# pranoyr/attention-models

Hardware: AMD Instinct MI355X
Metric: ViTVQGAN 256px train-step images/sec (higher is better)
Workload: dtype f32; 1 GPU; BASELINE.json configs[2]: ViTVQGAN dim=256 patch=8 img=256 depth=6+6 h=8 d=64 mlp=2048 (SwiGLU), codebook 8192x32; GAN train step (D phase + G phase, gradient penalty, per_loss_weight=0), Adam, clip 1.0; global_batch=32, batch_per_gpu=32, parallelism=dp1

## Files before the change

### attention-models_amd/amk/dense.py

```python
import ctypes

import torch

from . import lib as _lib
from .lib import EPI_BIAS, EPI_RESID, EPI_SWIGLU, EPI_SWIGLU_BWD, GEMM_NN, GEMM_NT, GEMM_TN, GemmDesc


def _p(t):
    return ctypes.c_void_p(t.data_ptr()) if t is not None else ctypes.c_void_p(0)


def _stream():
    return ctypes.c_void_p(torch.cuda.current_stream().cuda_stream)


def _mat(t, what):
    if t is None:
        return None
    if not t.is_cuda:
        raise RuntimeError("amk ops run only on MI355X (HIP) tensors; got a CPU tensor. There is no CPU fallback.")
    if t.dtype != torch.float32:
        raise RuntimeError(f"amk kernels compute in fp32; got {t.dtype} for {what}")
    if t.dim() != 2:
        raise RuntimeError(f"{what} must be a matrix, got shape {tuple(t.shape)}")
    if t.stride(1) != 1 or t.stride(0) % 4 or t.data_ptr() % 16:
        t = t.contiguous()
    return t


def _vec(t, n, what):
    if t is None:
        return None
    if not t.is_cuda or t.dtype != torch.float32:
        raise RuntimeError(f"{what}: an fp32 HIP tensor is required")
    t = t.contiguous()
    if t.numel() != n:
        raise RuntimeError(f"{what}: {t.numel()} elements, expected {n}")
    return t


def supported(*dims):
    return all(d > 0 and d % 4 == 0 for d in dims)


def _run(d, ws=None):
    L = _lib.load()
    rc = L.amk_gemm_f32(ctypes.byref(d), _p(ws), ws.numel() * 4 if ws is not None else 0, _stream())
    _lib.check(rc, "amk_gemm_f32")


def _set_ln(d, ln, M, K):
    if ln is None:
        return ()
    mean, rstd, gamma, beta = ln
    keep = (_vec(mean, M, "ln mean"), _vec(rstd, M, "ln rstd"), _vec(gamma, K, "ln gamma"), _vec(beta, K, "ln beta"))
    d.ln_mean, d.ln_rstd, d.ln_gamma, d.ln_beta = (_p(t) for t in keep)
    return keep


def row_stats(x2, eps=1e-5):
    x2 = _mat(x2, "x")
    M, D = x2.shape
    if x2.stride(0) != D:
        x2 = x2.contiguous()
    mean = torch.empty((M,), device=x2.device, dtype=torch.float32)
    rstd = torch.empty_like(mean)
    _lib.check(_lib.load().amk_row_stats(_p(x2), M, D, float(eps), _p(mean), _p(rstd), _stream()), "amk_row_stats")
    return mean, rstd


def gemm_nt(a, w, bias=None, *, w2=None, bias2=None, resid=None, ln=None, out=None):
    a, w, w2, resid = _mat(a, "a"), _mat(w, "w"), _mat(w2, "w2"), _mat(resid, "resid")
    M, K = a.shape
    N1 = w.shape[0]
    N2 = w2.shape[0] if w2 is not None else 0
    if w.shape[1] != K or (w2 is not None and w2.shape[1] != K):
        raise RuntimeError(f"gemm_nt: a {tuple(a.shape)} against w {tuple(w.shape)}")
    c = out if out is not None else torch.empty((M, N1), device=a.device, dtype=torch.float32)
    c2 = torch.empty((M, N2), device=a.device, dtype=torch.float32) if w2 is not None else None
    d = GemmDesc(op=GEMM_NT, epilogue=EPI_RESID if resid is not None else EPI_BIAS, m=M, n=N1 + N2, k=K,
                 split=N1 if w2 is not None else 0)
    bias, bias2 = _vec(bias, N1, "bias"), _vec(bias2, N2, "bias2")
    d.a, d.lda, d.w, d.ldw, d.c, d.ldc, d.bias = _p(a), a.stride(0), _p(w), w.stride(0), _p(c), c.stride(0), _p(bias)
    if w2 is not None:
        d.w2, d.ldw2, d.c2, d.ldc2, d.bias2 = _p(w2), w2.stride(0), _p(c2), c2.stride(0), _p(bias2)
    if resid is not None:
        if resid.shape != (M, N1):
            raise RuntimeError(f"gemm_nt: resid {tuple(resid.shape)} against output {(M, N1)}")
        d.resid, d.ldr = _p(resid), resid.stride(0)
    keep = _set_ln(d, ln, M, K)
    _run(d)
    return (c, c2) if w2 is not None else c


def gemm_nt_swiglu(a, w12, b12=None, *, ln=None, keep_ab=True):
    a, w12 = _mat(a, "a"), _mat(w12, "w12")
    M, K = a.shape
    H = w12.shape[0] // 2
    if w12.shape[1] != K or w12.shape[0] != 2 * H:
        raise RuntimeError(f"gemm_nt_swiglu: a {tuple(a.shape)} against w12 {tuple(w12.shape)}")
    gate = torch.empty((M, H), device=a.device, dtype=torch.float32)
    ab = torch.empty((M, 2 * H), device=a.device, dtype=torch.float32) if keep_ab else None
    d = GemmDesc(op=GEMM_NT, epilogue=EPI_SWIGLU, m=M, n=H, k=K)
    b12 = _vec(b12, 2 * H, "b12")
    d.a, d.lda, d.w, d.ldw, d.bias = _p(a), a.stride(0), _p(w12), w12.stride(0), _p(b12)
    d.gate, d.ldg = _p(gate), H
    d.c, d.ldc = _p(ab), 2 * H
    keep = _set_ln(d, ln, M, K)
    _run(d)
    return gate, ab


def gemm_nn(a, w, *, a2=None, w2=None, swiglu_ab=None):
    a, w, a2, w2, swiglu_ab = _mat(a, "a"), _mat(w, "w"), _mat(a2, "a2"), _mat(w2, "w2"), _mat(swiglu_ab, "ab")
    M, K1 = a.shape
    N = w.shape[1]
    K2 = a2.shape[1] if a2 is not None else 0
    if w.shape[0] != K1 or (a2 is not None and (w2 is None or w2.shape != (K2, N) or a2.shape[0] != M)):
        raise RuntimeError(f"gemm_nn: a {tuple(a.shape)} against w {tuple(w.shape)}")
    width = 2 * N if swiglu_ab is not None else N
    c = torch.empty((M, width), device=a.device, dtype=torch.float32)
    d = GemmDesc(op=GEMM_NN, epilogue=EPI_SWIGLU_BWD if swiglu_ab is not None else EPI_BIAS, m=M, n=N, k=K1 + K2,
                 split=K1 if a2 is not None else 0)
    d.a, d.lda, d.w, d.ldw, d.c, d.ldc = _p(a), a.stride(0), _p(w), w.stride(0), _p(c), width
    if a2 is not None:
        d.a2, d.lda2, d.w2, d.ldw2 = _p(a2), a2.stride(0), _p(w2), w2.stride(0)
    if swiglu_ab is not None:
        if swiglu_ab.shape != (M, 2 * N):
            raise RuntimeError(f"gemm_nn: (a | b) {tuple(swiglu_ab.shape)} against dGate {(M, N)}")
        d.ab, d.ldab = _p(swiglu_ab), swiglu_ab.stride(0)
    _run(d)
    return c


def _out(t, shape, what):
    if t is None:
        return None
    if (not t.is_cuda or t.dtype != torch.float32 or tuple(t.shape) != tuple(shape) or not t.is_contiguous()
            or t.data_ptr() % 16):
        raise RuntimeError(f"{what}: an fp32 contiguous 16-byte aligned HIP tensor of shape {tuple(shape)} is required")
    return t


def gemm_tn(y, x, *, y2=None, ln=None, want_bias=False, out=None, out2=None, bias_out=None):
    y, x, y2 = _mat(y, "y"), _mat(x, "x"), _mat(y2, "y2")
    M, N1 = y.shape
    K = x.shape[1]
    N2 = y2.shape[1] if y2 is not None else 0
    if x.shape[0] != M or (y2 is not None and y2.shape[0] != M):
        raise RuntimeError(f"gemm_tn: y {tuple(y.shape)} against x {tuple(x.shape)}")
    dw = _out(out, (N1, K), "gemm_tn out")
    if dw is None:
        dw = torch.empty((N1, K), device=y.device, dtype=torch.float32)
    dw2 = None
    if y2 is not None:
        dw2 = _out(out2, (N2, K), "gemm_tn out2")
        if dw2 is None:
            dw2 = torch.empty((N2, K), device=y.device, dtype=torch.float32)
    db = None
    if want_bias:
        db = _out(bias_out, (N1 + N2,), "gemm_tn bias_out")
        if db is None:
            db = torch.empty((N1 + N2,), device=y.device, dtype=torch.float32)
    d = GemmDesc(op=GEMM_TN, epilogue=EPI_BIAS, m=M, n=N1 + N2, k=K, split=N1 if y2 is not None else 0)
    d.a, d.lda, d.w, d.ldw, d.c, d.ldc, d.dbias = _p(y), y.stride(0), _p(x), x.stride(0), _p(dw), K, _p(db)
    if y2 is not None:
        d.a2, d.lda2, d.c2, d.ldc2 = _p(y2), y2.stride(0), _p(dw2), K
    keep = _set_ln(d, ln, M, K)
    L = _lib.load()
    nbytes = L.amk_gemm_f32_ws_bytes(ctypes.byref(d))
    ws = torch.empty((nbytes // 4,), device=y.device, dtype=torch.float32) if nbytes else None
    _run(d, ws)
    return dw, dw2, db


def _mat16(t, what):
    if not t.is_cuda:
        raise RuntimeError("amk ops run only on MI355X (HIP) tensors; got a CPU tensor. There is no CPU fallback.")
    if t.dtype != torch.bfloat16 or t.dim() != 2:
        raise RuntimeError(f"{what} must be a bf16 matrix, got {t.dtype} {tuple(t.shape)}")
    if t.stride(1) != 1 or t.stride(0) % 8 or t.data_ptr() % 16:
        t = t.contiguous()
    return t


def supported_bf16(N, K):
    return N > 0 and K > 0 and N % 8 == 0 and K % 8 == 0


def gemm_tn_bf16(y, x, want_bias=False, out=None, bias_out=None):
    y, x = _mat16(y, "y"), _mat16(x, "x")
    M, N = y.shape
    K = x.shape[1]
    if x.shape[0] != M:
        raise RuntimeError(f"gemm_tn_bf16: y has {M} rows, x {x.shape[0]}")
    if not supported_bf16(N, K):
        raise RuntimeError(f"gemm_tn_bf16: N and K must be multiples of 8, got {N}, {K}")
    L = _lib.load()
    dw = _out(out, (N, K), "gemm_tn_bf16 out")
    if dw is None:
        dw = torch.empty(N, K, device=y.device, dtype=torch.float32)
    db = None
    if want_bias:
        db = _out(bias_out, (N,), "gemm_tn_bf16 bias_out")
        if db is None:
            db = torch.empty(N, device=y.device, dtype=torch.float32)
    nbytes = L.amk_gemm_tn_bf16_ws_bytes(M, N, K)
    ws = torch.empty(nbytes // 4, device=y.device, dtype=torch.float32) if nbytes else None
    rc = L.amk_gemm_tn_bf16(_p(y), y.stride(0), _p(x), x.stride(0), _p(dw), K, _p(db), M, N, K, _p(ws), nbytes, _stream())
    _lib.check(rc, "amk_gemm_tn_bf16")
    return dw, db


def _bias32(bias, n):
    if bias is None:
        return None
    if bias.dtype != torch.float32 or not bias.is_cuda:
        raise RuntimeError("gemm bf16: the bias stays in fp32 (it is added to the fp32 accumulators)")
    bias = bias.contiguous()
    if bias.numel() != n or bias.data_ptr() % 16:
        raise RuntimeError(f"gemm bf16: bias of {bias.numel()} elements (16-byte aligned) expected {n}")
    return bias


def gemm_nt_bf16(a, w, bias=None):
    a, w = _mat16(a, "a"), _mat16(w, "w")
    (M, K), N = a.shape, w.shape[0]
    if w.shape[1] != K or not supported_bf16(N, K):
        raise RuntimeError(f"gemm_nt_bf16: a {tuple(a.shape)} x w {tuple(w.shape)}^T (multiples of 8 required)")
    bias = _bias32(bias, N)
    c = torch.empty(M, N, device=a.device, dtype=torch.bfloat16)
    if M:
        rc = _lib.load().amk_gemm_bf16(0, 0, _p(a), a.stride(0), _p(w), w.stride(0), _p(bias), _p(c), N, _p(None), 0, M, N, K, _stream())
        _lib.check(rc, "amk_gemm_bf16")
    return c


def gemm_nn_bf16(a, w):
    a, w = _mat16(a, "a"), _mat16(w, "w")
    (M, K), N = a.shape, w.shape[1]
    if w.shape[0] != K or not supported_bf16(N, K):
        raise RuntimeError(f"gemm_nn_bf16: a {tuple(a.shape)} x w {tuple(w.shape)} (multiples of 8 required)")
    c = torch.empty(M, N, device=a.device, dtype=torch.bfloat16)
    if M:
        rc = _lib.load().amk_gemm_bf16(1, 0, _p(a), a.stride(0), _p(w), w.stride(0), _p(None), _p(c), N, _p(None), 0, M, N, K, _stream())
        _lib.check(rc, "amk_gemm_bf16")
    return c


def gemm_nt_swiglu_bf16(a, w12, b12=None, keep_ab=True):
    a, w12 = _mat16(a, "a"), _mat16(w12, "w12")
    (M, K), N = a.shape, w12.shape[0]
    if w12.shape[1] != K or N % 16 or K % 8:
        raise RuntimeError(f"gemm_nt_swiglu_bf16: a {tuple(a.shape)} x w12 {tuple(w12.shape)}^T (2 H a multiple of 16, K of 8)")
    b12 = _bias32(b12, N)
    g = torch.empty(M, N // 2, device=a.device, dtype=torch.bfloat16)
    ab = torch.empty(M, N, device=a.device, dtype=torch.bfloat16) if keep_ab else None
    if M:
        rc = _lib.load().amk_gemm_bf16(0, 1, _p(a), a.stride(0), _p(w12), w12.stride(0), _p(b12), _p(ab), N, _p(g), N // 2, M, N, K, _stream())
        _lib.check(rc, "amk_gemm_bf16")
    return g, ab


def gemm_nn_swiglu_bwd_bf16(dy, w3, ab):
    dy, w3, ab = _mat16(dy, "dy"), _mat16(w3, "w3"), _mat16(ab, "ab")
    (M, K), H = dy.shape, w3.shape[1]
    if w3.shape[0] != K or ab.shape != (M, 2 * H) or not supported_bf16(H, K):
        raise RuntimeError(f"gemm_nn_swiglu_bwd_bf16: dy {tuple(dy.shape)}, w3 {tuple(w3.shape)}, ab {tuple(ab.shape)}")
    dab = torch.empty(M, 2 * H, device=dy.device, dtype=torch.bfloat16)
    if M:
        rc = _lib.load().amk_gemm_bf16_swiglu_bwd(_p(dy), dy.stride(0), _p(w3), w3.stride(0), _p(ab), ab.stride(0), _p(dab), 2 * H,
                                                  M, H, K, _stream())
        _lib.check(rc, "amk_gemm_bf16_swiglu_bwd")
    return dab
```

### attention-models_amd/amk/lib.py

```python
import ctypes
import os
import re

_HERE = os.path.dirname(os.path.abspath(__file__))
LIB_PATH = os.environ.get("AMK_LIB") or os.path.join(_HERE, "libamk.so")
HEADER_PATH = os.path.normpath(os.path.join(_HERE, "..", "..", "include", "amk.h"))

AMK_OK = 0

_c = ctypes
_P = _c.c_void_p
_I = _c.c_int
_L = _c.c_int64
_F = _c.c_float



class GemmDesc(_c.Structure):
    _fields_ = [("op", _c.c_int32), ("epilogue", _c.c_int32), ("m", _L),
                ("n", _c.c_int32), ("k", _c.c_int32), ("split", _c.c_int32), ("reserved", _c.c_int32),
                ("a", _P), ("a2", _P), ("w", _P), ("w2", _P), ("c", _P), ("c2", _P),
                ("lda", _L), ("lda2", _L), ("ldw", _L), ("ldw2", _L), ("ldc", _L), ("ldc2", _L),
                ("bias", _P), ("bias2", _P), ("resid", _P), ("ldr", _L),
                ("ln_mean", _P), ("ln_rstd", _P), ("ln_gamma", _P), ("ln_beta", _P),
                ("ab", _P), ("ldab", _L), ("gate", _P), ("ldg", _L), ("dbias", _P)]


GEMM_NT, GEMM_NN, GEMM_TN = 0, 1, 2
EPI_BIAS, EPI_RESID, EPI_SWIGLU, EPI_SWIGLU_BWD = 0, 1, 2, 3

SIGNATURES = {
    "amk_version": (_I, []),
    "amk_arch": (_c.c_char_p, []),
    "amk_last_error": (_c.c_char_p, []),
    "amk_attn_fwd": (_I, [_P] * 7 + [_I] * 5 + [_L] * 12 + [_F, _P]),
    "amk_attn_scores_bytes": (_L, [_I, _I, _I, _I]),
    "amk_attn_fwd_keep": (_I, [_P] * 8 + [_I] * 5 + [_L] * 12 + [_F, _P]),
    "amk_attn_fwd_x6_ws_bytes": (_L, [_I, _I, _I]),
    "amk_attn_fwd_x6": (_I, [_P] * 8 + [_I] * 5 + [_L] * 12 + [_F, _P]),
    "amk_attn_fwd_x6_keep": (_I, [_P] * 9 + [_I] * 5 + [_L] * 12 + [_F, _P]),
    "amk_attn_decode_ws_floats": (_L, [_I, _I, _I, _I]),
    "amk_attn_decode": (_I, [_P] * 9 + [_I] * 4 + [_L] * 9 + [_F, _P]),
    "amk_attn_decode_bf16": (_I, [_P] * 9 + [_I] * 4 + [_L] * 9 + [_F, _P]),
    "amk_gemm_rows_bf16": (_I, [_P, _L, _P, _L, _P, _P, _L, _I, _I, _I, _I, _P]),
    "amk_attn_bwd_ws_floats": (_L, [_I, _I, _I, _I, _I]),
    "amk_attn_bwd": (_I, [_P] * 12 + [_I] * 5 + [_L] * 24 + [_F, _I, _P]),
    "amk_attn_bwd_kept": (_I, [_P] * 13 + [_I] * 5 + [_L] * 24 + [_F, _I, _P]),
    "amk_vq_num_partials": (_L, [_L]),
    "amk_vq_lookup_fwd": (_I, [_P, _P, _L, _I, _I, _I] + [_P] * 9 + [_P]),
    "amk_vq_lookup_bwd": (_I, [_P] * 7 + [_F, _L, _I, _I, _P, _P, _P]),
    "amk_vq_lookup_bwd_rows": (_I, [_P] * 7 + [_F, _L, _I, _I, _P, _P, _P]),
    "amk_vq_padded_codes": (_I, [_I, _I]),
    "amk_vq_gather": (_I, [_P, _P, _L, _I, _I, _P, _P, _P]),
    "amk_agent_num_chunks": (_I, [_I]),
    "amk_agent_ws_floats": (_L, [_I, _I, _I, _I, _I]),
    "amk_agent_num_chunks_dh": (_I, [_I, _I]),
    "amk_agent_ws_floats_dh": (_L, [_I, _I, _I, _I, _I, _I]),
    "amk_agent_attn_fwd": (_I, [_P] * 10 + [_I] * 5 + [_L] * 12 + [_F, _P]),
    "amk_agent_attn_bwd": (_I, [_P] * 14 + [_I] * 5 + [_L] * 21 + [_F, _P]),
    "amk_agent_conv_grad_reduce": (_I, [_P, _P, _L, _I, _P, _P, _P]),
    "amk_rowsum_num_partials": (_I, [_L]),
    "amk_add_layernorm_fwd": (_I, [_P, _P, _P, _P, _L, _I, _F, _P, _P, _P, _P, _P]),
    "amk_add_layernorm_bwd": (_I, [_P, _P, _P, _P, _P, _P, _L, _I, _P, _P, _P]),
    "amk_colsum": (_I, [_P, _L, _I, _P, _P]),
    "amk_swiglu_fwd": (_I, [_P, _L, _I, _P, _P]),
    "amk_swiglu_bwd": (_I, [_P, _P, _L, _I, _P, _P]),
    "amk_geglu_fwd": (_I, [_P, _L, _I, _P, _P]),
    "amk_geglu_bwd": (_I, [_P, _P, _L, _I, _P, _P]),
    "amk_opt_num_partials": (_I, []),
    "amk_sumsq_partials": (_I, [_P, _L, _P, _P]),
    "amk_adam_flat_step": (_I, [_P] * 4 + [_L, _P, _P, _P, _I] + [_F] * 6 + [_I, _P, _P]),
    "amk_adam_flat_step_shadow": (_I, [_P] * 4 + [_L, _P, _P, _P, _I] + [_F] * 6 + [_I, _P, _P, _P]),
    "amk_gemm_x6_planes_bytes": (_L, [_I, _I]),
    "amk_gemm_x6_split": (_I, [_P, _L, _I, _I, _P, _P]),
    "amk_gemm_x6_nt": (_I, [_P, _L, _P, _P, _P, _L, _I, _I, _I, _P]),
    "amk_gemm_f32_ws_bytes": (_L, [_c.POINTER(GemmDesc)]),
    "amk_gemm_f32": (_I, [_c.POINTER(GemmDesc), _P, _L, _P]),
    "amk_row_stats": (_I, [_P, _L, _I, _F, _P, _P, _P]),
    "amk_attn_bf16_fwd": (_I, [_P] * 7 + [_I] * 5 + [_L] * 12 + [_F, _P]),
    "amk_attn_bf16_bwd_ws_floats": (_L, [_I, _I, _I, _I]),
    "amk_attn_bf16_bwd": (_I, [_P] * 12 + [_I] * 5 + [_L] * 24 + [_F, _P]),
    "amk_swiglu_bf16_fwd": (_I, [_P, _L, _I, _P, _P]),
    "amk_swiglu_bf16_bwd": (_I, [_P, _P, _L, _I, _P, _P]),
    "amk_add_layernorm_mixed_fwd": (_I, [_P, _I, _P, _P, _P, _L, _I, _F, _P, _P, _P, _P, _P]),
    "amk_add_layernorm_mixed_bwd": (_I, [_P, _I, _P, _P, _P, _P, _P, _L, _I, _P, _P, _P, _P]),
    "amk_geglu_ln_bf16_num_partials": (_I, [_L, _I]),
    "amk_geglu_ln_bf16_fwd": (_I, [_P, _L, _L, _I, _P, _P, _F, _P, _P, _P, _P]),
    "amk_geglu_ln_bf16_bwd": (_I, [_P, _L, _P, _P, _P, _P, _L, _I, _P, _P, _P]),
    "amk_gemm_bf16": (_I, [_I, _I, _P, _L, _P, _L, _P, _P, _L, _P, _L, _L, _I, _I, _P]),
    "amk_gemm_bf16_swiglu_bwd": (_I, [_P, _L, _P, _L, _P, _L, _P, _L, _L, _I, _I, _P]),
    "amk_gemm_tn_bf16_ws_bytes": (_L, [_L, _I, _I]),
    "amk_gemm_tn_bf16": (_I, [_P, _L, _P, _L, _P, _L, _P, _L, _I, _I, _P, _L, _P]),
    "amk_sample_step": (_I, [_P, _P, _F, _P, _c.c_uint64, _c.c_uint64, _F, _L, _I, _I, _P, _F, _P, _P, _P]),
    "amk_moe_route_ws_ints": (_L, [_L, _I, _I]),
    "amk_moe_route": (_I, [_P, _L, _I, _I] + [_P] * 8),
    "amk_grouped_gemm_nt": (_I, [_P, _L, _I, _P, _P, _P, _P, _L, _I, _I, _I, _P, _P]),
    "amk_grouped_gemm_nn": (_I, [_P, _L, _I, _P, _P, _P, _P, _L, _I, _I, _I, _P, _P]),
    "amk_grouped_gemm_nt_acc": (_I, [_P, _L, _I, _P, _P, _P, _P, _L, _I, _I, _I, _P, _I, _P]),
    "amk_grouped_gemm_nn_acc": (_I, [_P, _L, _I, _P, _P, _P, _P, _L, _I, _I, _I, _P, _I, _P]),
    "amk_grouped_gemm_wgrad": (_I, [_P, _L, _I, _P, _L, _I, _P, _P, _P, _L, _I, _I, _I, _P, _P, _P]),
    "amk_moe_combine": (_I, [_P, _P, _P, _L, _I, _I, _I, _P, _P]),
    "amk_moe_expert_sums": (_I, [_P, _L, _I, _P, _P, _L, _I, _I, _I, _P, _P]),
    "amk_moe_topk": (_I, [_P, _L, _I, _I, _P, _P, _P]),
    "amk_moe_route_distinct": (_I, [_P, _L, _I, _I, _P, _P, _P, _P]),
    "amk_moe_combine_rows": (_I, [_P, _P, _P, _L, _I, _I, _I, _I, _I, _P, _P]),
    "amk_moe_gate_grad_rows": (_I, [_P, _P, _P, _P, _L, _I, _I, _I, _I, _I, _P, _P]),
    "amk_moe_gate_grad": (_I, [_P, _P, _P, _P, _L, _I, _I, _I, _I, _P, _P]),
    "amk_bnact_ws_floats": (_L, [_I, _I, _L]),
    "amk_bnact_fwd": (_I, [_P, _P, _P, _I, _I, _L, _F, _F, _F] + [_P] * 7),
    "amk_bnact_bwd": (_I, [_P] * 6 + [_I, _I, _L, _F] + [_P] * 6),
    "amk_bnact_bwd_bwd": (_I, [_P] * 10 + [_I, _I, _L, _F] + [_P] * 5),
    "amk_bnact_bf16_fwd": (_I, [_P, _P, _P, _I, _I, _L, _F, _F, _F] + [_P] * 7),
    "amk_bnact_bf16_bwd": (_I, [_P] * 6 + [_I, _I, _L, _F] + [_P] * 6),
    "amk_bnact_bf16_bwd_bwd": (_I, [_P] * 10 + [_I, _I, _L, _F] + [_P] * 5),
    "amk_gnact_ws_floats": (_L, [_I, _I, _L, _I]),
    "amk_gnact_fwd": (_I, [_P, _P, _P, _I, _I, _L, _I, _F, _I] + [_P] * 5),
    "amk_gnact_bwd": (_I, [_P] * 6 + [_I, _I, _L, _I, _I] + [_P] * 5),
    "amk_gnact_bf16_ws_floats": (_L, [_I, _I, _L, _I]),
    "amk_gnact_bf16_fwd": (_I, [_P, _P, _P, _I, _I, _L, _I, _F, _I] + [_P] * 5),
    "amk_gnact_bf16_bwd": (_I, [_P] * 6 + [_I, _I, _L, _I, _I] + [_P] * 5),
    "amk_ce_head_fwd_ws_bytes": (_L, [_L, _I, _I]),
    "amk_ce_head_bwd_ws_bytes": (_L, [_L, _I, _I]),
    "amk_ce_head_fwd": (_I, [_P, _L, _P, _L, _P, _L, _L, _I, _I, _P, _P, _P, _P, _P, _L, _P]),
    "amk_ce_head_bwd": (_I, [_P, _L, _P, _L, _P, _L, _L, _I, _I, _P, _P, _P, _P, _P, _L, _P, _L, _P, _L, _P]),
    "amk_ce_head_bias_fwd": (_I, [_P, _L, _P, _L, _P, _P, _L, _L, _I, _I, _P, _P, _P, _P, _P, _L, _P]),
    "amk_ce_head_bias_bwd": (_I, [_P, _L, _P, _L, _P, _P, _L, _L, _I, _I, _P, _P, _P, _P, _P, _L, _P, _L, _P, _P, _L, _P]),
    "amk_ce_head_bf16_fwd_ws_bytes": (_L, [_L, _I, _I]),
    "amk_ce_head_bf16_bwd_ws_bytes": (_L, [_L, _I, _I]),
    "amk_ce_head_bf16_fwd": (_I, [_P, _L, _P, _L, _P, _L, _L, _I, _I, _P, _P, _P, _P, _P, _L, _P]),
    "amk_ce_head_bf16_bwd": (_I, [_P, _L, _P, _L, _P, _L, _L, _I, _I, _P, _P, _P, _P, _P, _L, _P, _L, _P, _L, _P]),
    "amk_ce_head_bias_bf16_fwd": (_I, [_P, _L, _P, _L, _P, _P, _L, _L, _I, _I, _P, _P, _P, _P, _P, _L, _P]),
    "amk_ce_head_bias_bf16_bwd": (_I, [_P, _L, _P, _L, _P, _P, _L, _L, _I, _I, _P, _P, _P, _P, _P, _L, _P, _L, _P, _P, _L, _P]),
    "amk_grouped_gemm_nt_bf16": (_I, [_P, _L, _I, _P, _P, _P, _P, _L, _I, _I, _I, _P, _P]),
    "amk_grouped_gemm_nn_bf16": (_I, [_P, _L, _I, _P, _P, _P, _P, _L, _I, _I, _I, _P, _P]),
    "amk_grouped_gemm_wgrad_bf16": (_I, [_P, _L, _I, _P, _L, _I, _P, _P, _P, _L, _I, _I, _I, _P, _P, _P]),
    "amk_grouped_gemm_nt64_bf16": (_I, [_P, _L, _I, _P, _P, _P, _P, _L, _I, _I, _I, _P, _P]),
    "amk_grouped_gemm_nn64_bf16": (_I, [_P, _L, _I, _P, _P, _P, _P, _L, _I, _I, _I, _P, _P]),
    "amk_grouped_gemm_wgrad64_bf16": (_I, [_P, _L, _I, _P, _L, _I, _P, _P, _P, _L, _I, _I, _I, _P, _P]),
    "amk_moe_expert_sums_bf16": (_I, [_P, _I, _L, _I, _P, _P, _L, _I, _I, _I, _P, _P]),
}

_lib = None


def declared_symbols(header_path=HEADER_PATH):
    text = open(header_path).read()
    text = re.sub(r"/\*.*?\*/", "", text, flags=re.S)
    return sorted(set(re.findall(r"\b(amk_[a-z0-9_]+)\s*\(", text)))


def load():
    global _lib
    if _lib is not None:
        return _lib
    if not os.path.exists(LIB_PATH):
        raise RuntimeError(
            f"{LIB_PATH} is missing: build it with `python -c 'import __graft_entry__ as g; g.build()'` "
            "(hipcc --offload-arch=gfx950). amk has no CPU or eager fallback."
        )
    lib = ctypes.CDLL(LIB_PATH)
    for name, (res, args) in SIGNATURES.items():
        fn = getattr(lib, name)
        fn.restype = res
        fn.argtypes = args
    arch = lib.amk_arch().decode()
    if arch != "gfx950":
        raise RuntimeError(f"libamk.so was built for {arch}, expected gfx950")
    _lib = lib
    return lib


def check(rc, what):
    if rc != AMK_OK:
        msg = load().amk_last_error().decode()
        raise RuntimeError(f"{what} failed with code {rc}: {msg}")
```

### attention-models_amd/amk/ops.py

```python
import ctypes
import os
import weakref

import torch
from torch.autograd.function import once_differentiable

from . import lib as _lib

_NULL = ctypes.c_void_p(0)


def _ptr(t):
    return ctypes.c_void_p(t.data_ptr()) if t is not None else _NULL


def _stream():
    return ctypes.c_void_p(torch.cuda.current_stream().cuda_stream)


KERNEL_EVENTS = None


class _timed:

# ... 1185 lines not shown

def agent_attention(qkv2, conv_w, conv_b, num_heads, dim_head, pool, scale):
    return _AgentAttn.apply(qkv2, conv_w, conv_b, num_heads, dim_head, pool, scale)


def _c16(t):
    t = t.contiguous()
    return t if t.data_ptr() % 16 == 0 else t.clone()


class _SwiGLU(torch.autograd.Function):
    FWD, BWD = "amk_swiglu_fwd", "amk_swiglu_bwd"

    @classmethod
    def forward(cls, ctx, ab):
        _require_device(ab)
        H = ab.shape[-1] // 2
        ab2 = _c16(ab).view(-1, 2 * H)
        M = ab2.shape[0]
        out = torch.empty((M, H), device=ab.device, dtype=torch.float32)
        L = _lib.load()
        _lib.check(getattr(L, cls.FWD)(_ptr(ab2), M, H, _ptr(out), _stream()), cls.FWD)
        ctx.save_for_backward(ab2)
        ctx.shape = ab.shape
        return out.view(*ab.shape[:-1], H)

    @classmethod
    def backward(cls, ctx, d_out):
        (ab2,) = ctx.saved_tensors
        M, H2 = ab2.shape
        d_out = _c16(d_out).view(M, H2 // 2)
        d_ab = torch.empty_like(ab2)
        L = _lib.load()
        _lib.check(getattr(L, cls.BWD)(_ptr(ab2), _ptr(d_out), M, H2 // 2, _ptr(d_ab), _stream()), cls.BWD)
        return d_ab.view(ctx.shape)


class _GEGLU(_SwiGLU):
    FWD, BWD = "amk_geglu_fwd", "amk_geglu_bwd"


def _f32_outside_autocast(fn, x, act):
    if x.shape[-1] % 8 != 0:
        a, b = x.chunk(2, dim=-1)
        return act(a) * b
    if torch.is_autocast_enabled():
        with torch.autocast("cuda", enabled=False):
            return fn(x.float())
    return fn(x)


class _SwiGLUBF16(torch.autograd.Function):

    @staticmethod
    def forward(ctx, ab):
        H = ab.shape[-1] // 2
        ab2 = ab.contiguous().view(-1, 2 * H)
        M = ab2.shape[0]
        out = torch.empty((M, H), device=ab.device, dtype=torch.bfloat16)
        _lib.check(_lib.load().amk_swiglu_bf16_fwd(_ptr(ab2), M, H, _ptr(out), _stream()), "amk_swiglu_bf16_fwd")
        ctx.save_for_backward(ab2)
        ctx.shape = ab.shape
        return out.view(*ab.shape[:-1], H)

    @staticmethod
    @once_differentiable
    def backward(ctx, d_out):
        (ab2,) = ctx.saved_tensors
        M, H2 = ab2.shape
        d_out = d_out.to(torch.bfloat16).contiguous().view(M, H2 // 2)
        d_ab = torch.empty_like(ab2)
        _lib.check(_lib.load().amk_swiglu_bf16_bwd(_ptr(ab2), _ptr(d_out), M, H2 // 2, _ptr(d_ab), _stream()), "amk_swiglu_bf16_bwd")
        return d_ab.view(ctx.shape)


MIXED_ELEMENTWISE = os.environ.get("AMK_MIXED_ELEMENTWISE", "1") == "1"


def swiglu(ab):
    if MIXED_ELEMENTWISE and ab.dtype == torch.bfloat16 and ab.is_cuda and ab.shape[-1] % 8 == 0:
        with torch.autocast("cuda", enabled=False):
            return _SwiGLUBF16.apply(ab)
    return _f32_outside_autocast(_SwiGLU.apply, ab, torch.nn.functional.silu)


def geglu(ab):
    return _f32_outside_autocast(_GEGLU.apply, ab, torch.nn.functional.gelu)


def _ln_supported(D):
    return 0 < D <= 4096 and D % 4 == 0


def _ln_param_grads(part, params):
    weight, bias = params if params is not None else (None, None)
    (wr, wv), (br, bv) = _claim_late(weight), _claim_late(bias)
    if wv is None and bv is None:
        dgb = part.sum(0)
        return dgb[0], dgb[1]
    dw = db = None
    if wv is not None:
        torch.sum(part[:, 0], dim=0, out=wv)
        wr.wrote(weight)
    else:
        dw = part[:, 0].sum(0)
    if bv is not None:
        torch.sum(part[:, 1], dim=0, out=bv)
        br.wrote(bias)
    else:
        db = part[:, 1].sum(0)
    return dw, db


def _claim_late(p):
    return _claim(p)


def _ln_backward(dy, h, dh_in, weight, mean, rstd, params=None):
    M, D = h.shape
    L = _lib.load()
    dh = torch.empty_like(h)
    part = torch.empty((L.amk_rowsum_num_partials(M), 2, D), device=h.device, dtype=torch.float32)
    _lib.check(L.amk_add_layernorm_bwd(_ptr(dy), _ptr(h), _ptr(dh_in), _ptr(weight), _ptr(mean), _ptr(rstd),
                                       M, D, _ptr(dh), _ptr(part), _stream()), "amk_add_layernorm_bwd")
    dw, db = _ln_param_grads(part, params)
    return dh, dw, db


class _LayerNorm(torch.autograd.Function):
    @staticmethod
    @_amp_fwd
    def forward(ctx, x, weight, bias, eps):
        _require_device(x, weight, bias)
        D = x.shape[-1]
        x2 = _c16(x).view(-1, D)
        M = x2.shape[0]
        y = torch.empty_like(x2)
        mean = torch.empty((M,), device=x.device, dtype=torch.float32)
        rstd = torch.empty_like(mean)
        w, b = _c16(weight), _c16(bias)
        L = _lib.load()
        _lib.check(L.amk_add_layernorm_fwd(_ptr(x2), _NULL, _ptr(w), _ptr(b), M, D, float(eps), _NULL, _ptr(y),
                                           _ptr(mean), _ptr(rstd), _stream()), "amk_add_layernorm_fwd")
        ctx.save_for_backward(x2, w, mean, rstd)
        ctx.shape = x.shape
        ctx.params = (weight, bias)
        return y.view(x.shape)

    @staticmethod
    @once_differentiable
    @_amp_bwd
    def backward(ctx, dy):
        x2, w, mean, rstd = ctx.saved_tensors
        dx, dw, db = _ln_backward(_c16(dy).view(x2.shape), x2, None, w, mean, rstd, ctx.params)
        return dx.view(ctx.shape), dw, db, None


class _AddLayerNorm(torch.autograd.Function):

    @staticmethod
    @_amp_fwd
    def forward(ctx, x, res, weight, bias, eps):
        _require_device(x, res, weight, bias)
        D = x.shape[-1]
        x2 = _c16(x).view(-1, D)
        r2 = _c16(res).view(-1, D)
        M = x2.shape[0]
        h = torch.empty_like(x2)
        y = torch.empty_like(x2)
        mean = torch.empty((M,), device=x.device, dtype=torch.float32)
        rstd = torch.empty_like(mean)
        w, b = _c16(weight), _c16(bias)
        L = _lib.load()
        _lib.check(L.amk_add_layernorm_fwd(_ptr(x2), _ptr(r2), _ptr(w), _ptr(b), M, D, float(eps), _ptr(h), _ptr(y),
                                           _ptr(mean), _ptr(rstd), _stream()), "amk_add_layernorm_fwd")
        ctx.save_for_backward(h, w, mean, rstd)
        ctx.shape = x.shape
        ctx.params = (weight, bias)
        ctx.set_materialize_grads(False)
        return h.view(x.shape), y.view(x.shape)

    @staticmethod
    @once_differentiable
    @_amp_bwd
    def backward(ctx, dh_in, dy):
        h, w, mean, rstd = ctx.saved_tensors
        if dy is None:
            if dh_in is None:
                return None, None, None, None, None
            return dh_in, dh_in, None, None, None
        dh2 = _c16(dh_in).view(h.shape) if dh_in is not None else None
        dh, dw, db = _ln_backward(_c16(dy).view(h.shape), h, dh2, w, mean, rstd, ctx.params)
        dh = dh.view(ctx.shape)
        return dh, dh, dw, db, None


class _AddLayerNormMixed(torch.autograd.Function):

    @staticmethod
    def forward(ctx, x, res, weight, bias, eps):
        _require_device(res, weight, bias)
        D = x.shape[-1]
        x2 = x.contiguous().view(-1, D)
        M = x2.shape[0]
        xb = x2.dtype == torch.bfloat16
        if not xb and x2.dtype != torch.float32:
            raise RuntimeError(f"mixed LayerNorm takes f32 or bf16 inputs, got {x2.dtype}")
        r2 = res.contiguous().view(-1, D) if res is not None else None
        need_h = r2 is not None or xb
        h = torch.empty((M, D), device=x.device, dtype=torch.float32) if need_h else None
        y = torch.empty((M, D), device=x.device, dtype=torch.bfloat16)
        mean = torch.empty((M,), device=x.device, dtype=torch.float32)
        rstd = torch.empty_like(mean)
        w, b = weight.contiguous(), bias.contiguous()
        _lib.check(_lib.load().amk_add_layernorm_mixed_fwd(_ptr(x2), 1 if xb else 0, _ptr(r2), _ptr(w), _ptr(b), M, D, float(eps),
                                                          _ptr(h), _ptr(y), _ptr(mean), _ptr(rstd), _stream()),
                   "amk_add_layernorm_mixed_fwd")
        hs = h if need_h else x2
        ctx.save_for_backward(hs, w, mean, rstd)
        ctx.cfg = (x.shape, xb, res is not None)
        ctx.params = (weight, bias)
        ctx.set_materialize_grads(False)
        return hs.view(x.shape), y.view(x.shape)

    @staticmethod
    @once_differentiable
    def backward(ctx, dh_in, dy):
        h, w, mean, rstd = ctx.saved_tensors
        shape, xb, has_res = ctx.cfg
        M, D = h.shape
        if dy is None:
            if dh_in is None:
                return None, None, None, None, None
            dx = dh_in.to(torch.bfloat16) if xb else dh_in
            return dx, (dh_in if has_res else None), None, None, None
        dyb = dy.dtype == torch.bfloat16
        dy2 = (dy if dyb else dy.float()).contiguous().view(M, D)
        dh2 = dh_in.float().contiguous().view(M, D) if dh_in is not None else None
        L = _lib.load()
        dh = torch.empty((M, D), device=h.device, dtype=torch.float32)
        dh16 = torch.empty((M, D), device=h.device, dtype=torch.bfloat16) if xb else None
        part = torch.empty((L.amk_rowsum_num_partials(M), 2, D), device=h.device, dtype=torch.float32)
        _lib.check(L.amk_add_layernorm_mixed_bwd(_ptr(dy2), 1 if dyb else 0, _ptr(h), _ptr(dh2), _ptr(w), _ptr(mean), _ptr(rstd),
                                                 M, D, _ptr(dh), _ptr(dh16), _ptr(part), _stream()), "amk_add_layernorm_mixed_bwd")
        dw, db = _ln_param_grads(part, ctx.params)
        dhv = dh.view(shape)
        dx = dh16.view(shape) if xb else dhv
        return dx, (dhv if has_res else None), dw, db, None


def _mixed_ln():
    return (MIXED_ELEMENTWISE and torch.is_autocast_enabled() and torch.get_autocast_dtype("cuda") == torch.bfloat16)


def layer_norm(x, weight, bias, eps=1e-5, branch=False):
    if not _ln_supported(x.shape[-1]) or x.numel() == 0 or not x.is_cuda:
        return torch.nn.functional.layer_norm(x, (x.shape[-1],), weight, bias, eps)
    if branch and _mixed_ln():
        with torch.autocast("cuda", enabled=False):
            return _AddLayerNormMixed.apply(x, None, weight, bias, eps)[1]
    return _LayerNorm.apply(x, weight, bias, eps)


def add_layer_norm(x, res, weight, bias, eps=1e-5, branch=False):
    if not _ln_supported(x.shape[-1]) or x.numel() == 0 or not x.is_cuda:
        h = x + res
        return h, torch.nn.functional.layer_norm(h, (h.shape[-1],), weight, bias, eps)
    if branch and _mixed_ln():
        with torch.autocast("cuda", enabled=False):
            return _AddLayerNormMixed.apply(x, res.float(), weight, bias, eps)
    return _AddLayerNorm.apply(x, res, weight, bias, eps)


def colsum(x2):
    M, N = x2.shape
    if N % 4 != 0 or N > 1024:
        return x2.sum(0)
    x2 = _c16(x2)
    L = _lib.load()
    part = torch.empty((L.amk_rowsum_num_partials(M), N), device=x2.device, dtype=torch.float32)
    _lib.check(L.amk_colsum(_ptr(x2), M, N, _ptr(part), _stream()), "amk_colsum")
    return part.sum(0)


class _BiasLinear(torch.autograd.Function):

    @staticmethod
    def forward(ctx, x, weight, bias):
        _require_device(x, weight, bias)
        ctx.save_for_backward(x, weight)
        return torch.nn.functional.linear(x, weight, bias)

    @staticmethod
    @once_differentiable
    def backward(ctx, dy):
        x, weight = ctx.saved_tensors
        dy2 = dy.contiguous().view(-1, dy.shape[-1])
        dx = dy2.mm(weight).view(x.shape) if ctx.needs_input_grad[0] else None
        dw = dy2.t().mm(x.reshape(-1, x.shape[-1])) if ctx.needs_input_grad[1] else None
        db = colsum(dy2) if ctx.needs_input_grad[2] else None
        return dx, dw, db


GEMM_MODE = os.environ.get("AMK_GEMM", "f32")


def gemm_x6_nt(a2, b2, bias=None):
    _require_device(a2, b2, bias)
    if a2.stride(1) != 1:
        a2 = a2.contiguous()
    if b2.stride(1) != 1:
        b2 = b2.contiguous()
    M, K = a2.shape
    N = b2.shape[0]
    L = _lib.load()
    planes = torch.empty((L.amk_gemm_x6_planes_bytes(N, K),), device=a2.device, dtype=torch.uint8)
    c = torch.empty((M, N), device=a2.device, dtype=torch.float32)
    with _timed(f"gemm_x6_nt M{M} N{N} K{K}"):
        _lib.check(L.amk_gemm_x6_split(_ptr(b2), b2.stride(0), N, K, _ptr(planes), _stream()), "amk_gemm_x6_split")
        rc = L.amk_gemm_x6_nt(_ptr(a2), a2.stride(0), _ptr(planes), _ptr(bias), _ptr(c), N, M, N, K, _stream())
    _lib.check(rc, "amk_gemm_x6_nt")
    return c


def _x6_ok(x, weight):
    K = weight.shape[1]
    if K % 4 or x.numel() == 0 or x.data_ptr() % 16 or weight.data_ptr() % 16:
        return False
    if x.stride(-1) != 1 or (x.dim() >= 2 and x.stride(-2) % 4):
        return False
    return x.numel() * 4 < 0x7ffffff0 and weight.numel() * 8 < 0x7ffffff0


class _LinearX6(torch.autograd.Function):

    @staticmethod
    def forward(ctx, x, weight, bias):
        _require_device(x, weight, bias)
        x2 = x.reshape(-1, x.shape[-1])
        ctx.save_for_backward(x2, weight)
        ctx.x_shape = x.shape
        ctx.has_bias = bias is not None
        return gemm_x6_nt(x2, weight, bias).view(*x.shape[:-1], weight.shape[0])

    @staticmethod
    @once_differentiable
    def backward(ctx, dy):
        x2, weight = ctx.saved_tensors
        dy2 = dy.contiguous().view(-1, dy.shape[-1])
        dx = dw = db = None
        if ctx.needs_input_grad[0]:
            N = weight.shape[0]
            if N % 4 == 0:
                dx = gemm_x6_nt(dy2, weight.t().contiguous()).view(ctx.x_shape)
            else:
                dx = dy2.mm(weight).view(ctx.x_shape)
        if ctx.needs_input_grad[1]:
            dw = dy2.t().mm(x2)
        if ctx.has_bias and ctx.needs_input_grad[2]:
            db = colsum(dy2)
        return dx, dw, db


DENSE_MODE = os.environ.get("AMK_DENSE", "auto")


DENSE_AUTO_MAX_K = int(os.environ.get("AMK_DENSE_MAX_K", "512"))


def _dense_ok(x, *weights):
    if DENSE_MODE == "lib" or torch.is_autocast_enabled() or not x.is_cuda or x.dtype != torch.float32 or x.numel() == 0:
        return False
    if x.shape[-1] % 4 or x.shape[-1] < 128:
        return False
    if DENSE_MODE == "auto" and x.shape[-1] > DENSE_AUTO_MAX_K:
        return False
    return all(w.dtype == torch.float32 and w.shape[0] % 4 == 0 and w.shape[0] >= 128 and w.is_contiguous() for w in weights)


def _nn_plain(dy2, weight):
    from . import dense

    if DENSE_MODE == "amk":
        return dense.gemm_nn(dy2, weight)
    return dy2.mm(weight)


def _claim(p):
    ref = getattr(p, "_amk_reducer", None) if p is not None else None
    red = ref() if ref is not None else None
    if red is None:
        return None, None
    view = red.claim(p)
    return (red, view) if view is not None else (None, None)


class _DenseLinear(torch.autograd.Function):

    @staticmethod
    def forward(ctx, x, weight, bias):
        from . import dense

        x2 = x.reshape(-1, x.shape[-1])
        ctx.save_for_backward(x2, weight)
        ctx.x_shape = x.shape
        ctx.has_bias = bias is not None
        ctx.params = (weight, bias)
        if DENSE_MODE == "auto" and weight.shape[0] < 512:
            return torch.nn.functional.linear(x, weight, bias)
        return dense.gemm_nt(x2, weight, bias).view(*x.shape[:-1], weight.shape[0])

    @staticmethod
    @once_differentiable
    def backward(ctx, dy):
        from . import dense

        x2, weight = ctx.saved_tensors
        dy2 = dy.reshape(-1, dy.shape[-1])
        dx = dw = db = None
        if ctx.needs_input_grad[0]:
            dx = _nn_plain(dy2, weight).view(ctx.x_shape)
        if ctx.needs_input_grad[1] or (ctx.has_bias and ctx.needs_input_grad[2]):
            want_b = ctx.has_bias and ctx.needs_input_grad[2]
            (wr, wv), (br, bv) = _claim(ctx.params[0]), (_claim(ctx.params[1]) if want_b else (None, None))
            dw, _, db = dense.gemm_tn(dy2, x2, want_bias=want_b, out=wv, bias_out=bv)
            if wv is not None:
                wr.wrote(ctx.params[0])
                dw = None
            if bv is not None:
                br.wrote(ctx.params[1])
                db = None
        return dx, dw, db


def _tn_into(tn, y, x, weight, bias):
    (wr, wv), (br, bv) = _claim(weight), _claim(bias)
    res = tn(y, x, want_bias=bias is not None, out=wv, bias_out=bv)
    dw, db = res[0], res[-1]
    if wv is not None:
        wr.wrote(weight)
        dw = None
    if bv is not None:
        br.wrote(bias)
        db = None
    return dw, db


class _DenseLinear2(torch.autograd.Function):

    @staticmethod
    def forward(ctx, x, wa, wb):
        from . import dense

        x2 = x.reshape(-1, x.shape[-1])
        ctx.save_for_backward(x2, wa, wb)
        ctx.x_shape = x.shape
        ctx.params = (wa, wb)
        a, b = dense.gemm_nt(x2, wa, None, w2=wb)
        return a.view(*x.shape[:-1], wa.shape[0]), b.view(*x.shape[:-1], wb.shape[0])

    @staticmethod
    @once_differentiable
    def backward(ctx, da, db_):
        from . import dense

        x2, wa, wb = ctx.saved_tensors
        da2 = da.reshape(-1, da.shape[-1])
        db2 = db_.reshape(-1, db_.shape[-1])
        dx = dense.gemm_nn(da2, wa, a2=db2, w2=wb).view(ctx.x_shape) if ctx.needs_input_grad[0] else None
        dwa = dwb = None
        if ctx.needs_input_grad[1] or ctx.needs_input_grad[2]:
            (ar, av), (br, bv) = _claim(ctx.params[0]), _claim(ctx.params[1])
            dwa, dwb, _ = dense.gemm_tn(da2, x2, y2=db2, out=av, out2=bv)
            if av is not None:
                ar.wrote(ctx.params[0])
                dwa = None
            if bv is not None:
                br.wrote(ctx.params[1])
                dwb = None
        return dx, dwa, dwb


class _SwiGLUFFN(torch.autograd.Function):

    @staticmethod
    def forward(ctx, x, w12, b12, w3, b3):
        from . import dense

        x2 = x.reshape(-1, x.shape[-1])
        need = any(ctx.needs_input_grad)
        gate, ab = dense.gemm_nt_swiglu(x2, w12, b12, keep_ab=need)
        out = dense.gemm_nt(gate, w3, b3)
        if need:
            ctx.save_for_backward(x2, w12, w3, ab, gate)
        ctx.x_shape = x.shape
        ctx.has_bias = (b12 is not None, b3 is not None)
        ctx.params = (w12, b12, w3, b3)
        return out.view(*x.shape[:-1], w3.shape[0])

    @staticmethod
    @once_differentiable
    def backward(ctx, dout):
        from . import dense

        x2, w12, w3, ab, gate = ctx.saved_tensors
        d2 = dout.reshape(-1, dout.shape[-1])
        d_ab = dense.gemm_nn(d2, w3, swiglu_ab=ab)
        dw3, db3 = _tn_into(dense.gemm_tn, d2, gate, ctx.params[2], ctx.params[3] if ctx.has_bias[1] else None)
        dx = _nn_plain(d_ab, w12).view(ctx.x_shape) if ctx.needs_input_grad[0] else None
        dw12, db12 = _tn_into(dense.gemm_tn, d_ab, x2, ctx.params[0], ctx.params[1] if ctx.has_bias[0] else None)
        return dx, dw12, db12, dw3, db3


MIXED_WGRAD = os.environ.get("AMK_MIXED_WGRAD", "1") == "1"


def _w16(t):
    if t is None:
        return None
    shadow = getattr(t, "_amk_bf16", None)
    if shadow is not None and t._version == t._amk_bf16_version:
        return shadow
    return t.to(torch.bfloat16)


class _LinearMixed(torch.autograd.Function):

    @staticmethod
    def forward(ctx, x, weight, bias):
        x16, w16 = x.to(torch.bfloat16), _w16(weight)
        ctx.save_for_backward(x16, w16)
        ctx.has_bias, ctx.x_dtype = bias is not None, x.dtype
        ctx.params = (weight, bias)
        return torch.nn.functional.linear(x16, w16, _w16(bias))

    @staticmethod
    @once_differentiable
    def backward(ctx, dy):
        from . import dense

        x16, w16 = ctx.saved_tensors
        dy2 = dy.reshape(-1, dy.shape[-1])
        dx = dy2.mm(w16).view(x16.shape).to(ctx.x_dtype) if ctx.needs_input_grad[0] else None
        dw, db = _tn_into(dense.gemm_tn_bf16, dy2, x16.reshape(-1, x16.shape[-1]), ctx.params[0], ctx.params[1])
        return dx, dw, db


def _mixed_linear_ok(x, weight):
    return (MIXED_WGRAD and x.is_cuda and torch.get_autocast_dtype("cuda") == torch.bfloat16 and torch.is_grad_enabled()
            and weight.requires_grad and weight.dtype == torch.float32 and x.dtype in (torch.float32, torch.bfloat16)
            and weight.shape[0] % 8 == 0 and weight.shape[1] % 8 == 0 and x.numel() > 0)


def linear(x, weight, bias=None):
    if torch.is_autocast_enabled():
        if _mixed_linear_ok(x, weight):
            return _LinearMixed.apply(x, weight, bias)
        return torch.nn.functional.linear(x, weight, bias)
    if GEMM_MODE == "bf16x6" and _x6_ok(x, weight):
        return _LinearX6.apply(x, weight, bias)
    if _dense_ok(x, weight):
        return _DenseLinear.apply(x, weight, bias)
    if bias is None:
        return torch.nn.functional.linear(x, weight)
    return _BiasLinear.apply(x, weight, bias)


def linear2(x, wa, wb):
    if GEMM_MODE != "bf16x6" and _dense_ok(x, wa, wb) and wa.shape[0] % 128 == 0:
        return _DenseLinear2.apply(x, wa, wb)
    return linear(x, wa), linear(x, wb)


class _SwiGLUFFNMixed(torch.autograd.Function):

    @staticmethod
    def forward(ctx, x, w12, b12, w3, b3):
        from . import dense

        x16 = x.to(torch.bfloat16).reshape(-1, x.shape[-1])
        w12h, w3h = _w16(w12), _w16(w3)
        g, ab = dense.gemm_nt_swiglu_bf16(x16, w12h, b12)
        y = torch.nn.functional.linear(g, w3h, _w16(b3))
        ctx.save_for_backward(x16, ab, g, w12h, w3h)
        ctx.x_shape, ctx.x_dtype, ctx.bias = x.shape, x.dtype, (b12 is not None, b3 is not None)
        ctx.params = (w12, b12, w3, b3)
        return y.view(*x.shape[:-1], w3.shape[0])

    @staticmethod
    @once_differentiable
    def backward(ctx, dy):
        from . import dense

        x16, ab, g, w12h, w3h = ctx.saved_tensors
        dy2 = dy.reshape(-1, dy.shape[-1])
        dw3, db3 = _tn_into(dense.gemm_tn_bf16, dy2, g, ctx.params[2], ctx.params[3])
        dab = dense.gemm_nn_swiglu_bwd_bf16(dy2, w3h, ab)
        dw12, db12 = _tn_into(dense.gemm_tn_bf16, dab, x16, ctx.params[0], ctx.params[1])
        dx = dab.mm(w12h).view(ctx.x_shape).to(ctx.x_dtype) if ctx.needs_input_grad[0] else None
        return dx, dw12, db12, dw3, db3


def swiglu_ffn(x, w12, b12, w3, b3):
    if torch.is_autocast_enabled() and w12.shape[0] % 16 == 0 and w12.shape[0] >= 1024:
        if _mixed_linear_ok(x, w12) and _mixed_linear_ok(x, w3) and w3.requires_grad:
            with torch.autocast("cuda", enabled=False):
                return _SwiGLUFFNMixed.apply(x, w12, b12, w3, b3)
        no_grad = not torch.is_grad_enabled() or not any(
            t is not None and t.requires_grad for t in (x, w12, b12, w3, b3))
        if (MIXED_WGRAD and no_grad and x.is_cuda and torch.get_autocast_dtype("cuda") == torch.bfloat16
                and w12.dtype == torch.float32 and x.dtype in (torch.float32, torch.bfloat16) and w12.shape[1] % 8 == 0 and x.numel()):
            from . import dense

            g, _ = dense.gemm_nt_swiglu_bf16(x.to(torch.bfloat16).reshape(-1, x.shape[-1]), _w16(w12), b12, keep_ab=False)
            return torch.nn.functional.linear(g, _w16(w3), _w16(b3)).view(*x.shape[:-1], w3.shape[0])
    if GEMM_MODE != "bf16x6" and _dense_ok(x, w12) and w3.shape[1] % 4 == 0 and w3.shape[0] % 4 == 0 and w3.is_contiguous():
        return _SwiGLUFFN.apply(x, w12, b12, w3, b3)
    ab = linear(x, w12, b12)
    if ab.shape[-1] % 8 == 0:
        return linear(swiglu(ab), w3, b3)
    a, b = ab.chunk(2, dim=-1)
    return linear(torch.nn.functional.silu(a) * b, w3, b3)


GEGLU_FFN_BF16 = os.environ.get("AMK_GEGLU_FFN_BF16", "1") != "0"


def geglu_ln_bf16_fwd(ab2, gamma, beta, eps=1e-5):
    M, H = ab2.shape[0], ab2.shape[1] // 2
    y = torch.empty((M, H), device=ab2.device, dtype=torch.bfloat16)
    mean = torch.empty((M,), device=ab2.device, dtype=torch.float32)
    rstd = torch.empty_like(mean)
    with _timed(f"geglu_ln_bf16_fwd M{M} H{H}"):
        _lib.check(_lib.load().amk_geglu_ln_bf16_fwd(_ptr(ab2), ab2.stride(0), M, H, _ptr(gamma), _ptr(beta), float(eps),
                                                     _ptr(y), _ptr(mean), _ptr(rstd), _stream()), "amk_geglu_ln_bf16_fwd")
    return y, mean, rstd


def geglu_ln_bf16_bwd(ab2, dy, gamma, mean, rstd):
    M, H = ab2.shape[0], ab2.shape[1] // 2
    L = _lib.load()
    d_ab = torch.empty((M, 2 * H), device=ab2.device, dtype=torch.bfloat16)
    part = torch.empty((L.amk_geglu_ln_bf16_num_partials(M, H), 2, H), device=ab2.device, dtype=torch.float32)
    with _timed(f"geglu_ln_bf16_bwd M{M} H{H}"):
        _lib.check(L.amk_geglu_ln_bf16_bwd(_ptr(ab2), ab2.stride(0), _ptr(dy), _ptr(gamma), _ptr(mean), _ptr(rstd), M, H,
                                           _ptr(d_ab), _ptr(part), _stream()), "amk_geglu_ln_bf16_bwd")
    return d_ab, part


class _GEGLUFFNMixed(torch.autograd.Function):

    @staticmethod
    def forward(ctx, x, w1, gamma, beta, w2, eps):
        x16 = x.to(torch.bfloat16).reshape(-1, x.shape[-1])
        w1h, w2h = _w16(w1), _w16(w2)
        gm, bt = gamma.contiguous(), beta.contiguous()
        ab = torch.nn.functional.linear(x16, w1h)
        y, mean, rstd = geglu_ln_bf16_fwd(ab, gm, bt, eps)
        out = torch.nn.functional.linear(y, w2h)
        if any(ctx.needs_input_grad):
            ctx.save_for_backward(x16, ab, y, mean, rstd, w1h, w2h, gm)
        ctx.x_shape, ctx.x_dtype = x.shape, x.dtype
        ctx.params = (w1, gamma, beta, w2)
        return out.view(*x.shape[:-1], w2.shape[0])

    @staticmethod
    @once_differentiable
    def backward(ctx, dy):
        from . import dense

        x16, ab, y, mean, rstd, w1h, w2h, gm = ctx.saved_tensors
        w1, gamma, beta, w2 = ctx.params
        dy2 = dy.to(torch.bfloat16).reshape(-1, dy.shape[-1])
        dw2, _ = _tn_into(dense.gemm_tn_bf16, dy2, y, w2, None)
        dyn = dy2.mm(w2h)
        d_ab, part = geglu_ln_bf16_bwd(ab, dyn, gm, mean, rstd)
        dgamma, dbeta = _ln_param_grads(part, (gamma, beta if ctx.needs_input_grad[3] else None))
        dw1, _ = _tn_into(dense.gemm_tn_bf16, d_ab, x16, w1, None)
        dx = d_ab.mm(w1h).view(ctx.x_shape).to(ctx.x_dtype) if ctx.needs_input_grad[0] else None
        return dx, dw1, dgamma, (dbeta if ctx.needs_input_grad[3] else None), dw2, None


def geglu_ffn_ok(x, w1, gamma, beta, w2):
    if not (GEGLU_FFN_BF16 and x.is_cuda and w1.is_cuda and w2.is_cuda and _bf16_autocast()):
        return False
    inner, dim = w2.shape[1], w2.shape[0]
    if not (w1.dtype == torch.float32 and w2.dtype == torch.float32 and gamma.dtype == torch.float32 and beta.dtype == torch.float32
            and x.dtype in (torch.float32, torch.bfloat16) and tuple(w1.shape) == (2 * inner, dim) and x.shape[-1] == dim
            and dim % 8 == 0 and inner % 8 == 0 and 8 <= inner <= 4096 and x.numel() > 0):
        return False
    if torch.is_grad_enabled() and any(t.requires_grad for t in (x, w1, gamma, beta, w2)):
        return w1.requires_grad and w2.requires_grad
    return True


def geglu_ffn(x, w1, gamma, beta, w2, eps=1e-5):
    if geglu_ffn_ok(x, w1, gamma, beta, w2):
        with torch.autocast("cuda", enabled=False):
            return _GEGLUFFNMixed.apply(x, w1, gamma, beta, w2, eps)
    ab = torch.nn.functional.linear(x, w1)
    if ab.is_cuda and ab.shape[-1] % 8 == 0 and ab.numel() > 0:
        g = geglu(ab)
    else:
        val, gate = ab.chunk(2, dim=-1)
        g = gate * torch.nn.functional.gelu(val)
    return torch.nn.functional.linear(layer_norm(g, gamma, beta, eps), w2)


def discr_norm_mode():
    return os.environ.get("AMK_DISCR_NORM", "amk")


def _bn_aligned(t):
    t = t.contiguous()
    return t if t.data_ptr() % 16 == 0 else t.clone()


def _bn_dims(x):
    N, C, H, W = x.shape
    return N, C, H * W


def _bn_ws(x):
    N, C, HW = _bn_dims(x)
    return torch.empty(int(_lib.load().amk_bnact_ws_floats(N, C, HW)), device=x.device, dtype=torch.float32)


class _BNActGrad(torch.autograd.Function):

    @staticmethod
    def forward(ctx, gz, x, weight, bias, mean, rstd, slope):
        gz = _bn_aligned(gz)
        N, C, HW = _bn_dims(x)
        L = _lib.load()
        gx = torch.empty_like(x)
        sums = torch.empty((2, C), device=x.device, dtype=torch.float32)
        dw = torch.empty_like(weight)
        db = torch.empty_like(bias)
        _lib.check(L.amk_bnact_bwd(_ptr(gz), _ptr(x), _ptr(weight), _ptr(bias), _ptr(mean), _ptr(rstd), N, C, HW,
                                   float(slope), _ptr(gx), _ptr(sums), _ptr(dw), _ptr(db), _ptr(_bn_ws(x)), _stream()),
                   "amk_bnact_bwd")
        ctx.save_for_backward(gz, x, weight, bias, mean, rstd, sums)
        ctx.slope = slope
        ctx.set_materialize_grads(False)
        return gx, dw, db

    @staticmethod
    @once_differentiable
    def backward(ctx, ggx, ggw, ggb):
        gz, x, weight, bias, mean, rstd, sums = ctx.saved_tensors
        if ggx is None and ggw is None and ggb is None:
            return None, None, None, None, None, None, None
        ggx = torch.zeros_like(x) if ggx is None else _bn_aligned(ggx)
        N, C, HW = _bn_dims(x)
        g_gz = torch.empty_like(x)
        g_x = torch.empty_like(x)
        g_w = torch.empty_like(weight) if ctx.needs_input_grad[2] else None
        _lib.check(_lib.load().amk_bnact_bwd_bwd(
            _ptr(ggx), _ptr(ggw.contiguous() if ggw is not None else None), _ptr(ggb.contiguous() if ggb is not None else None),
            _ptr(gz), _ptr(x), _ptr(weight), _ptr(bias), _ptr(mean), _ptr(rstd), _ptr(sums), N, C, HW, float(ctx.slope),
            _ptr(g_gz), _ptr(g_x), _ptr(g_w), _ptr(_bn_ws(x)), _stream()), "amk_bnact_bwd_bwd")
        return (g_gz if ctx.needs_input_grad[0] else None, g_x if ctx.needs_input_grad[1] else None, g_w,
                None, None, None, None)


class _BNAct(torch.autograd.Function):

    @staticmethod
    def forward(ctx, x, weight, bias, running_mean, running_var, eps, momentum, slope):
        N, C, HW = _bn_dims(x)
        L = _lib.load()
        z = torch.empty_like(x)
        mean = torch.empty(C, device=x.device, dtype=torch.float32)
        rstd = torch.empty(C, device=x.device, dtype=torch.float32)
        _lib.check(L.amk_bnact_fwd(_ptr(x), _ptr(weight), _ptr(bias), N, C, HW, float(eps), float(momentum), float(slope),
                                   _ptr(z), _ptr(mean), _ptr(rstd), _ptr(running_mean), _ptr(running_var),
                                   _ptr(_bn_ws(x)), _stream()), "amk_bnact_fwd")
        ctx.save_for_backward(x, weight, bias, mean, rstd)
        ctx.slope = slope
        ctx.set_materialize_grads(False)
        return z

    @staticmethod
    def backward(ctx, gz):
        if gz is None:
            return (None,) * 8
        x, weight, bias, mean, rstd = ctx.saved_tensors
        from .models.discriminator import input_grad_only_active

        gx, dw, db = _BNActGrad.apply(gz, x, weight, bias, mean, rstd, ctx.slope)
        if input_grad_only_active():
            dw = db = None
        return (gx if ctx.needs_input_grad[0] else None, dw if ctx.needs_input_grad[1] else None,
                db if ctx.needs_input_grad[2] else None, None, None, None, None, None)


def bn_leaky_relu_ok(bn, x):
    return (bn.training and bn.track_running_stats and bn.affine and bn.momentum is not None
            and bn.running_mean is not None and x.is_cuda and x.dtype == torch.float32 and x.dim() == 4
            and x.is_contiguous() and x.numel() > 0 and x.shape[0] * x.shape[2] * x.shape[3] > 1
            and not torch.is_autocast_enabled() and bn.weight.dtype == torch.float32)


def bn_leaky_relu(x, bn, slope):
    _require_device(x, bn.weight, bn.bias)
    if bn.num_batches_tracked is not None:
        bn.num_batches_tracked.add_(1)
    return _BNAct.apply(_bn_aligned(x), bn.weight, bn.bias, bn.running_mean, bn.running_var, bn.eps, bn.momentum,
                        float(slope))


def discr_norm_bf16_on():
    return os.environ.get("AMK_DISCR_NORM_BF16", "1") != "0"


def _bn_aligned_bf16(t):
    return _bn_aligned(t.to(torch.bfloat16))


def _bn_f32(t):
    return None if t is None else t.to(torch.float32).contiguous()


class _BNActGradBF16(torch.autograd.Function):

    @staticmethod
    def forward(ctx, gz, x, weight, bias, mean, rstd, slope):
        gz = _bn_aligned_bf16(gz)
        N, C, HW = _bn_dims(x)
        L = _lib.load()
        gx = torch.empty_like(x)
        sums = torch.empty((2, C), device=x.device, dtype=torch.float32)
        dw = torch.empty_like(weight)
        db = torch.empty_like(bias)
        _lib.check(L.amk_bnact_bf16_bwd(_ptr(gz), _ptr(x), _ptr(weight), _ptr(bias), _ptr(mean), _ptr(rstd), N, C, HW,
                                        float(slope), _ptr(gx), _ptr(sums), _ptr(dw), _ptr(db), _ptr(_bn_ws(x)),
                                        _stream()), "amk_bnact_bf16_bwd")
        ctx.save_for_backward(gz, x, weight, bias, mean, rstd, sums)
        ctx.slope = slope
        ctx.set_materialize_grads(False)
        return gx, dw, db

    @staticmethod
    @once_differentiable
    def backward(ctx, ggx, ggw, ggb):
        gz, x, weight, bias, mean, rstd, sums = ctx.saved_tensors
        if ggx is None and ggw is None and ggb is None:
            return None, None, None, None, None, None, None
        ggx = torch.zeros_like(x) if ggx is None else _bn_aligned_bf16(ggx)
        N, C, HW = _bn_dims(x)
        g_gz = torch.empty_like(x)
        g_x = torch.empty_like(x)
        g_w = torch.empty_like(weight) if ctx.needs_input_grad[2] else None
        _lib.check(_lib.load().amk_bnact_bf16_bwd_bwd(
            _ptr(ggx), _ptr(_bn_f32(ggw)), _ptr(_bn_f32(ggb)), _ptr(gz), _ptr(x), _ptr(weight), _ptr(bias), _ptr(mean),
            _ptr(rstd), _ptr(sums), N, C, HW, float(ctx.slope), _ptr(g_gz), _ptr(g_x), _ptr(g_w), _ptr(_bn_ws(x)),
            _stream()), "amk_bnact_bf16_bwd_bwd")
        return (g_gz if ctx.needs_input_grad[0] else None, g_x if ctx.needs_input_grad[1] else None, g_w,
                None, None, None, None)


class _BNActBF16(torch.autograd.Function):

    @staticmethod
    def forward(ctx, x, weight, bias, running_mean, running_var, eps, momentum, slope):
        N, C, HW = _bn_dims(x)
        L = _lib.load()
        z = torch.empty_like(x)
        mean = torch.empty(C, device=x.device, dtype=torch.float32)
        rstd = torch.empty(C, device=x.device, dtype=torch.float32)
        _lib.check(L.amk_bnact_bf16_fwd(_ptr(x), _ptr(weight), _ptr(bias), N, C, HW, float(eps), float(momentum),
                                        float(slope), _ptr(z), _ptr(mean), _ptr(rstd), _ptr(running_mean),
                                        _ptr(running_var), _ptr(_bn_ws(x)), _stream()), "amk_bnact_bf16_fwd")
        ctx.save_for_backward(x, weight, bias, mean, rstd)
        ctx.slope = slope
        ctx.set_materialize_grads(False)
        return z

    @staticmethod
    def backward(ctx, gz):
        if gz is None:
            return (None,) * 8
        x, weight, bias, mean, rstd = ctx.saved_tensors
        from .models.discriminator import input_grad_only_active

        gx, dw, db = _BNActGradBF16.apply(gz, x, weight, bias, mean, rstd, ctx.slope)
        if input_grad_only_active():
            dw = db = None
        return (gx if ctx.needs_input_grad[0] else None, dw if ctx.needs_input_grad[1] else None,
                db if ctx.needs_input_grad[2] else None, None, None, None, None, None)


def bn_leaky_relu_bf16_ok(bn, x):
    return (discr_norm_mode() == "amk" and discr_norm_bf16_on() and isinstance(bn, torch.nn.BatchNorm2d)
            and bn.training and bn.track_running_stats and bn.affine and bn.momentum is not None
            and bn.running_mean is not None and bn.running_mean.dtype == torch.float32
            and bn.weight.dtype == torch.float32 and bn.bias.dtype == torch.float32 and bn.weight.is_cuda
            and x.is_cuda and x.dtype == torch.bfloat16 and x.dim() == 4 and x.is_contiguous() and x.numel() > 0
            and x.shape[0] * x.shape[2] * x.shape[3] > 1)


def bn_leaky_relu_bf16(x, bn, slope):
    _require_device(bn.weight, bn.bias)
    if not x.is_cuda or x.dtype != torch.bfloat16:
        raise RuntimeError(f"bn_leaky_relu_bf16 takes a bf16 HIP tensor; got {x.dtype} on {x.device}")
    if bn.num_batches_tracked is not None:
        bn.num_batches_tracked.add_(1)
    return _BNActBF16.apply(_bn_aligned(x), bn.weight, bn.bias, bn.running_mean, bn.running_var, bn.eps, bn.momentum,
                            float(slope))


GN_ACT = os.environ.get("AMK_GN_ACT", "1") != "0"


def _gn_ws(x, G):
    N, C, HW = _bn_dims(x)
    return torch.empty(int(_lib.load().amk_gnact_ws_floats(N, C, HW, G)), device=x.device, dtype=torch.float32)

# ... 234 lines not shown
```

### attention-models_amd/amk/optim.py

```python
import ctypes
import os

import numpy as np
import torch

from . import lib as _lib
from .dp import ALIGN


def _ptr(t):
    return ctypes.c_void_p(t.data_ptr()) if t is not None else ctypes.c_void_p(0)


class FlatAdam:
    TABLE_WD = os.environ.get("AMK_OPT_TABLE_WD", "1") == "1"

    def __init__(self, reducer, lr=1e-3, betas=(0.9, 0.999), eps=1e-8, weight_decay=0.0, decoupled=False,
                 capturable=False, bf16_shadow=False, no_decay=()):
        if not reducer.on_gpu:
            raise RuntimeError("FlatAdam runs on MI355X (HIP) parameters only; use torch.optim on CPU")
        self.red = reducer
        self.capturable = bool(capturable)
        self._lr = float(lr)
        self.betas, self.eps, self.weight_decay, self.decoupled = betas, eps, weight_decay, decoupled
        self.L = _lib.load()
        self.npart = self.L.amk_opt_num_partials()
        dev = reducer.buckets[0].flat.device
        self.params = [p for b in reducer.buckets for p in b.params]
        self.steps = np.zeros(len(self.params), dtype=np.int64)
        skip = {id(p) for p in no_decay}
        self.wd = np.array([0.0 if id(p) in skip else float(weight_decay) for p in self.params], dtype=np.float64)
        self.flat_p, self.m, self.v, self.seg, self.flat_p16 = [], [], [], [], []
        pid = 0
        for b in reducer.buckets:
            fp = torch.zeros_like(b.flat)
            seg = torch.empty(b.flat.numel() // ALIGN, dtype=torch.int32)
            for p, off in zip(b.params, b.offsets):
                view = fp[off:off + p.numel()].view_as(p)
                view.copy_(p.data)
                p.data = view
                nseg = -(-p.numel() // ALIGN)
                seg[off // ALIGN: off // ALIGN + nseg] = pid
                pid += 1
            self.flat_p.append(fp)
            self.m.append(torch.zeros_like(b.flat))
            self.v.append(torch.zeros_like(b.flat))
            self.seg.append(seg.to(dev))
        if bf16_shadow:
            self.enable_shadow()
        else:
            self.disable_shadow()
        self.partials = torch.zeros(len(reducer.buckets) * self.npart, device=dev, dtype=torch.float32)
        self.norm = torch.zeros(1, device=dev, dtype=torch.float32)
        self._tab_host = [torch.zeros(len(self.params), 4).pin_memory() for _ in range(2)]
        self._tab_np = [t.numpy() for t in self._tab_host]
        self._tab_dev = [torch.zeros(len(self.params), 4, device=dev) for _ in range(2)]
        self._tab_done = [None, None]
        self._flip = 0
        if self.capturable:
            self.steps_dev = torch.zeros(len(self.params), device=dev, dtype=torch.float64)
            self.lr_dev = torch.full((), float(lr), device=dev, dtype=torch.float64)
            self._fired_host, self._fired_dev = None, None
            self.wd_dev = torch.tensor(self.wd, device=dev)

    def enable_shadow(self):
        if self.flat_p16:
            return self.refresh_shadow()
        for b, fp in zip(self.red.buckets, self.flat_p):
            f16 = fp.to(torch.bfloat16)
            for p, off in zip(b.params, b.offsets):
                p._amk_bf16 = f16[off:off + p.numel()].view_as(p)
                p._amk_bf16_version = p._version
            self.flat_p16.append(f16)

    def disable_shadow(self):
        for p in self.params:
            p.__dict__.pop("_amk_bf16", None)
            p.__dict__.pop("_amk_bf16_version", None)
        self.flat_p16 = []

    def refresh_shadow(self):
        for fp, f16 in zip(self.flat_p, self.flat_p16):
            f16.copy_(fp)
        if self.flat_p16:
            for p in self.params:
                p._amk_bf16_version = p._version

    @property
    def lr(self):
        return self._lr

    @lr.setter
    def lr(self, value):
        self._lr = float(value)
        if self.capturable:
            self.lr_dev.fill_(self._lr)

    def _device_table(self, fired):
        if self._fired_host is None or not np.array_equal(fired, self._fired_host):
            if torch.cuda.is_current_stream_capturing():
                raise RuntimeError("FlatAdam: the set of parameters with gradients changed inside a HIP-graph capture; "
                                   "run the step eagerly once (warm-up) before capturing")
            self._fired_host = fired.copy()
            self._fired_dev = torch.tensor(fired.astype(np.float64), device=self.steps_dev.device)
        b1, b2 = self.betas
        self.steps_dev += self._fired_dev
        t = self.steps_dev.clamp(min=1.0)
        tab = self._tab_dev[0]
        tab[:, 0] = self._fired_dev
        tab[:, 1] = self.lr_dev / (1.0 - torch.pow(torch.full_like(t, b1), t))
        tab[:, 2] = torch.sqrt(1.0 - torch.pow(torch.full_like(t, b2), t))
        tab[:, 3] = self.wd_dev * self.lr_dev if self.decoupled else self.wd_dev
        return tab

    def step(self, max_norm=None, lr=None):
        if lr is not None:
            self.lr = lr
        red, L = self.red, self.L
        stream = ctypes.c_void_p(torch.cuda.current_stream().cuda_stream)
        b1, b2 = self.betas
        fired = np.fromiter((f for b in red.buckets for f in b.fired), dtype=bool, count=len(self.params))
        if self.capturable:
            tab_d = self._device_table(fired)
        else:
            tab_h, tab_d = self._tab_host[self._flip], self._tab_dev[self._flip]
            if self._tab_done[self._flip] is not None:
                self._tab_done[self._flip].synchronize()
            done = self._tab_done[self._flip] = torch.cuda.Event()
            self._flip ^= 1
            self.steps += fired
            t = np.maximum(self.steps, 1).astype(np.float64)
            tab = self._tab_np[self._flip ^ 1]
            tab[:, 0] = fired
            tab[:, 1] = self.lr / (1.0 - b1 ** t)
            tab[:, 2] = np.sqrt(1.0 - b2 ** t)
            tab[:, 3] = self.wd * self.lr if self.decoupled else self.wd
            tab_d.copy_(tab_h, non_blocking=True)
            done.record()
        clip = float(max_norm) if max_norm else 0.0
        for k, b in enumerate(red.buckets):
            _lib.check(L.amk_sumsq_partials(_ptr(b.flat), b.flat.numel(), _ptr(self.partials[k * self.npart:]), stream),
                       "amk_sumsq_partials")
        for k, b in enumerate(red.buckets):
            rc = L.amk_adam_flat_step_shadow(
                _ptr(self.flat_p[k]), _ptr(b.flat), _ptr(self.m[k]), _ptr(self.v[k]), b.flat.numel(),
                _ptr(self.seg[k]), _ptr(tab_d), _ptr(self.partials), self.partials.numel(),
                clip, float(self.lr), float(b1), float(b2), float(self.eps), float(self.weight_decay),
                (2 if self.TABLE_WD else 0) | (1 if self.decoupled else 0), _ptr(self.norm) if k == 0 else _ptr(None),
                _ptr(self.flat_p16[k]) if self.flat_p16 else _ptr(None), stream)
            _lib.check(rc, "amk_adam_flat_step")
        red.mark_zeroed()
        return self.norm

    def state_of(self, p):
        k = next(i for i, q in enumerate(self.params) if q is p)
        bi = 0
        for b, m, v in zip(self.red.buckets, self.m, self.v):
            if k < bi + len(b.params):
                off = b.offsets[k - bi]
                step = int(self.steps_dev[k].item()) if self.capturable else int(self.steps[k])
                return dict(step=step, exp_avg=m[off:off + p.numel()].view_as(p),
                            exp_avg_sq=v[off:off + p.numel()].view_as(p))
            bi += len(b.params)
        raise KeyError("parameter not managed by this optimizer")
```

### attention-models_amd/amk/train.py

```python
import math

import torch
import torch.nn.functional as F

from .dp import GradReducer
from .models.discriminator import input_grad_only
from .optim import FlatAdam


def set_requires_grad(module, flag):
    for p in module.parameters():
        p.requires_grad_(flag)


def hinge_d_loss(fake, real):
    return 0.5 * (F.relu(1.0 - real).mean() + F.relu(1.0 + fake).mean())


def g_nonsaturating_loss(fake):
    return F.softplus(-fake).mean()


def cosine_warmup_lr(step, base_lr, t_initial, warmup_t, warmup_lr_init=1e-6, lr_min=5e-5):
    if step < warmup_t:
        return warmup_lr_init + step * (base_lr - warmup_lr_init) / warmup_t
    t = min(step, t_initial)
    return lr_min + 0.5 * (base_lr - lr_min) * (1.0 + math.cos(math.pi * t / t_initial))


def cosine_with_warmup_factor(step, num_warmup_steps, num_training_steps, num_cycles=0.5):
    if step < num_warmup_steps:
        return float(step) / float(max(1, num_warmup_steps))
    progress = float(step - num_warmup_steps) / float(max(1, num_training_steps - num_warmup_steps))
    return max(0.0, 0.5 * (1.0 + math.cos(math.pi * float(num_cycles) * 2.0 * progress)))


def constant_with_warmup_factor(step, num_warmup_steps):
    if step < num_warmup_steps:
        return float(step) / float(max(1.0, num_warmup_steps))
    return 1.0


class SupervisedTrainStep:

    def __init__(self, model, lr=1e-4, betas=(0.9, 0.999), weight_decay=0.01, no_decay=(), decoupled=True,
                 schedule="cosine_with_warmup", warmup_steps=0, total_steps=1, max_grad_norm=1.0, accum_steps=1,
                 autocast=None, capturable=False, bucket_bytes=32 << 20, fused_optimizer=None, direct_grads=None,
                 communicate_when_alone=False, overlap=True):
        self.model = model
        self.base_lr, self.schedule = float(lr), schedule
        self.warmup_steps, self.total_steps = int(warmup_steps), int(total_steps)
        self.max_grad_norm, self.accum_steps, self.autocast = max_grad_norm, int(accum_steps), autocast
        named = [(n, p) for n, p in model.named_parameters() if p.requires_grad]
        on_gpu = named[0][1].is_cuda
        self.red = GradReducer([p for _, p in named], bucket_bytes, communicate_when_alone=communicate_when_alone,
                               overlap=overlap, direct_grads=on_gpu if direct_grads is None else bool(direct_grads))
        skip = [p for n, p in named if any(frag in n for frag in no_decay)]
        self.fused_optimizer = on_gpu if fused_optimizer is None else bool(fused_optimizer)
        if self.fused_optimizer:
            self.optim = FlatAdam(self.red, lr=lr, betas=betas, weight_decay=weight_decay, decoupled=decoupled,
                                  capturable=capturable, bf16_shadow=autocast == torch.bfloat16, no_decay=skip)
        else:
            ids = {id(p) for p in skip}
            groups = [dict(params=[p for _, p in named if id(p) not in ids], weight_decay=weight_decay),
                      dict(params=skip, weight_decay=0.0)]
            cls = torch.optim.AdamW if decoupled else torch.optim.Adam
            kw = dict(capturable=True) if capturable else {}
            self.optim = cls([g for g in groups if g["params"]], betas=betas,
                             lr=torch.tensor(float(lr), device=named[0][1].device) if capturable else lr, **kw)
        self.red.broadcast_parameters()
        if self.fused_optimizer:
            self.optim.refresh_shadow()
        self.global_step = 0
        self._micro = 0
        self._lr_arg = 0
        self._graph = None
        self._accum_graph = None
        self.last_lr = None

    def _loss(self, *batch):
        raise NotImplementedError

    def lr_factor(self, step):
        if self.schedule == "cosine_with_warmup":
            return cosine_with_warmup_factor(step, self.warmup_steps, self.total_steps)
        if self.schedule == "constant_with_warmup":
            return constant_with_warmup_factor(step, self.warmup_steps)
        if self.schedule in (None, "constant"):
            return 1.0
        raise ValueError(f"unknown schedule {self.schedule!r}")

    def _set_lr(self):
        lr = self.last_lr = self.base_lr * self.lr_factor(self._lr_arg)
        if isinstance(self.optim, FlatAdam):
            self.optim.lr = lr
            return
        for g in self.optim.param_groups:
            if torch.is_tensor(g["lr"]):
                g["lr"].fill_(lr)
            else:
                g["lr"] = lr

    def _amp(self):
        import contextlib

        if self.autocast is None:
            return contextlib.nullcontext()
        dev = "cuda" if self.red.on_gpu else "cpu"
        return torch.autocast(dev, dtype=self.autocast)

    def step_body(self, sync, *batch):
        self.red.begin(sync)
        loss = self._loss(*batch)
        (loss if self.accum_steps == 1 else loss / self.accum_steps).backward()
        self.red.finish()
        if sync:
            if isinstance(self.optim, FlatAdam):
                self.optim.step(max_norm=self.max_grad_norm)
            else:
                if self.max_grad_norm:
                    torch.nn.utils.clip_grad_norm_(self.red.params, self.max_grad_norm)
                self.optim.step()
                self.red.zero_grad()
        return loss.detach()

    def step(self, *batch):
        self._micro += 1
        sync = self._micro % self.accum_steps == 0
        if sync:
            self._set_lr()
        g = self._graph
        if g is not None and sync and self.accum_steps == 1 and len(batch) == len(g.static_inputs) and all(
                a.shape == b.shape for a, b in zip(batch, g.static_inputs)):
            loss = g.replay(*batch)
        else:
            loss = self.step_body(sync, *batch)
        if sync:
            self._lr_arg = self.global_step
        self.global_step += 1
        return loss

    def _tick(self):
        self._micro += 1
        self._set_lr()
        self._lr_arg = self.global_step
        self.global_step += 1

    def capture(self, *batch, warmup=2):
        from .graphs import GraphedStep

        if self.accum_steps != 1:
            raise RuntimeError("capture(): gradient accumulation steps run eagerly")
        if not self.red.alone and not self.red.avg_in_collective:
            raise RuntimeError("capture(): only RCCL (backend 'nccl') collectives can be captured into a HIP graph")
        self._graph = None
        self._graph = GraphedStep(lambda *b: self.step_body(True, *b), list(batch), warmup=warmup, before_each=self._tick)

    def release_graph(self):
        self._graph = None
        self._accum_graph = None

    def _accum_body(self, k):
        n = self.accum_steps

        def body(*xs):
            for i in range(n - 1):
                self.step_body(False, *xs[i * k:(i + 1) * k])
            return self.step_body(True, *xs[(n - 1) * k:])
        return body

    def _tick_accum(self):
        n = self.accum_steps
        self._micro += n
        self._set_lr()
        self._lr_arg = self.global_step + n - 1
        self.global_step += n

    def capture_accumulated(self, micro_batches, warmup=2):
        from .graphs import GraphedStep

        if len(micro_batches) != self.accum_steps:
            raise ValueError(f"capture_accumulated: {len(micro_batches)} micro-batches for accum_steps={self.accum_steps}")
        if not self.red.alone and not self.red.avg_in_collective:
            raise RuntimeError("capture_accumulated(): only RCCL (backend 'nccl') collectives can be captured into a HIP graph")
        k = len(micro_batches[0])
        self._accum_graph = None
        self._accum_graph = GraphedStep(self._accum_body(k), [t for mb in micro_batches for t in mb], warmup=warmup,
                                        before_each=self._tick_accum)

    def step_accumulated(self, micro_batches):
        n = self.accum_steps
        if len(micro_batches) != n or self._micro % n != 0:
            raise ValueError("step_accumulated: pass accum_steps micro-batches, starting on an optimizer-step boundary")
        flat = [t for mb in micro_batches for t in mb]
        self._micro += n
        self._set_lr()
        g = getattr(self, "_accum_graph", None)
        if g is not None and len(flat) == len(g.static_inputs) and all(a.shape == b.shape for a, b in zip(flat, g.static_inputs)):
            loss = g.replay(*flat)
        else:
            loss = self._accum_body(len(micro_batches[0]))(*flat)
        self._lr_arg = self.global_step + n - 1
        self.global_step += n
        return loss

    def save_ckpt(self, path, config=None):
        import torch.distributed as dist

        if dist.is_initialized() and dist.get_rank() != 0:
            return
        torch.save({"step": self.global_step, "config": config,
                    "state_dict": {k: v.detach().cpu() for k, v in self.model.state_dict().items()}}, path)


    def resume_from_checkpoint(self, path):
        ckpt = torch.load(path, map_location="cpu", weights_only=True)
        self.global_step = int(ckpt["step"])
        self.model.load_state_dict(ckpt["state_dict"])
        self.red.broadcast_parameters()
        if self.fused_optimizer:
            self.optim.refresh_shadow()
        return ckpt.get("config")


class ClassifierTrainStep(SupervisedTrainStep):

    def _loss(self, imgs, target):
        with self._amp():
            out = self.model(imgs)
        return F.cross_entropy(out, target)


class MaskedTokenTrainStep(SupervisedTrainStep):

    NO_DECAY = ("bias", "layer_norm.weight", "embeddings.weight")

    def __init__(self, model, weight_decay=0.0, no_decay=NO_DECAY, schedule="constant_with_warmup", **kw):
        super().__init__(model, weight_decay=weight_decay, no_decay=no_decay, schedule=schedule, **kw)

    def _loss(self, *batch):
        with self._amp():
            return self.model(*batch)


class VQGANTrainStep:
    def __init__(self, model, discr, lr=1e-4, betas=(0.9, 0.999), weight_decay=0.0,
                 adv_loss_weight=0.1, logit_laplace_weight=1.0, max_grad_norm=1.0,
                 warmup_steps=50000, decay_steps=100000, gp_lambda=10.0, bucket_bytes=32 << 20,
                 share_forward=False, capturable=False, fused_optimizer=None, autocast=None, communicate_when_alone=False,
                 overlap=True):
        self.model, self.discr = model, discr
        self._autocast = autocast
        self.adv_w, self.laplace_w = adv_loss_weight, logit_laplace_weight
        self.max_grad_norm, self.gp_lambda = max_grad_norm, gp_lambda
        self.base_lr, self.warmup_steps, self.decay_steps = lr, warmup_steps, decay_steps
        fused = next(model.parameters()).is_cuda
        self.g_red = GradReducer(model.parameters(), bucket_bytes, direct_grads=fused, communicate_when_alone=communicate_when_alone,
                                 overlap=overlap)
        self.d_red = GradReducer(discr.parameters(), bucket_bytes, communicate_when_alone=communicate_when_alone, overlap=overlap)
        self.fused_optimizer = fused if fused_optimizer is None else bool(fused_optimizer)
        okw = dict(betas=betas, weight_decay=weight_decay, fused=fused)
        self._graph = None
        self._accum_graph = None
        if self.fused_optimizer:
            self.g_optim = FlatAdam(self.g_red, lr=lr, betas=betas, weight_decay=weight_decay, capturable=capturable,
                                    bf16_shadow=autocast == torch.bfloat16)
            self.d_optim = FlatAdam(self.d_red, lr=lr, betas=betas, weight_decay=weight_decay, capturable=capturable)
        elif capturable:
            dev = next(model.parameters()).device
            okw.update(capturable=True)
            self.g_optim = torch.optim.Adam(model.parameters(), lr=torch.tensor(float(lr), device=dev), **okw)
            self.d_optim = torch.optim.Adam(discr.parameters(), lr=torch.tensor(float(lr), device=dev), **okw)
        else:
            self.g_optim = torch.optim.Adam(model.parameters(), lr=lr, **okw)
            self.d_optim = torch.optim.Adam(discr.parameters(), lr=lr, **okw)
        self.g_red.broadcast_parameters()
        self.d_red.broadcast_parameters()
        if self.fused_optimizer:
            self.g_optim.refresh_shadow()
        self.global_step = 0
        self.share_forward = bool(share_forward)

    @property
    def autocast(self):
        return self._autocast

    @autocast.setter
    def autocast(self, dtype):
        self._autocast = dtype
        if self.fused_optimizer:
            if dtype == torch.bfloat16:
                self.g_optim.enable_shadow()
            else:
                self.g_optim.disable_shadow()

    def _amp(self):
        import contextlib

        if self.autocast is None:
            return contextlib.nullcontext()
        return torch.autocast("cuda", dtype=self.autocast)

    def gradient_penalty(self, real, fake, eta=None):
        if eta is None:
            eta = torch.rand(real.shape[0], 1, 1, 1, device=real.device)
        mixed = (eta * real + (1.0 - eta) * fake).detach().requires_grad_(True)
        pred = self.discr(mixed)
        with input_grad_only():
            (grad,) = torch.autograd.grad(pred, mixed, grad_outputs=torch.ones_like(pred),
                                          create_graph=True, retain_graph=True)
        return ((grad.norm(2, dim=1) - 1.0) ** 2).mean() * self.gp_lambda

    def _set_lr(self):
        lr = cosine_warmup_lr(max(self.global_step - 1, 0), self.base_lr, self.decay_steps, self.warmup_steps)
        for opt in (self.g_optim, self.d_optim):
            if isinstance(opt, FlatAdam):
                opt.lr = lr
                continue
            for g in opt.param_groups:
                if torch.is_tensor(g["lr"]):
                    g["lr"].fill_(lr)
                else:
                    g["lr"] = lr

    def step(self, img, sync=True, accum_steps=1, eta=None):
        self._set_lr()
        if self._graph is not None and sync and accum_steps == 1 and eta is None and img.shape == self._graph.static_inputs[0].shape:
            logs = self._graph.replay(img)
        else:
            logs = self.step_body(img, sync, accum_steps, eta)
        self.global_step += 1
        return logs

    def capture(self, img, warmup=2):
        from .graphs import GraphedStep

        self._check_capturable("capture")
        self._graph = None
        self._graph = GraphedStep(lambda x: self.step_body(x), [img], warmup=warmup, before_each=self._tick)

    def _check_capturable(self, what):
        for red in (self.g_red, self.d_red):
            if not red.alone and not red.avg_in_collective:
                raise RuntimeError(f"VQGANTrainStep.{what}: only RCCL (backend 'nccl') collectives can be captured into a "
                                   "HIP graph; over gloo the data-parallel step runs eagerly")

    def release_graph(self):
        self._graph = None
        self._accum_graph = None

    def capture_accumulated(self, micro_batches, warmup=2):
        from .graphs import GraphedStep

        self._check_capturable("capture_accumulated")
        n = len(micro_batches)

        def body(*xs):
            for x in xs[:-1]:
                self.step_body(x, False, n, None)
            return self.step_body(xs[-1], True, n, None)

        self._accum_graph = None
        self._accum_graph = GraphedStep(body, list(micro_batches), warmup=warmup, before_each=lambda: self._tick(n))

    def _tick(self, n=1):
        self.global_step += n - 1
        self._set_lr()
        self.global_step += 1

    def step_accumulated(self, micro_batches):
        self.global_step += len(micro_batches) - 1
        self._set_lr()
        self.global_step -= len(micro_batches) - 1
        g = getattr(self, "_accum_graph", None)
        if g is not None and len(micro_batches) == len(g.static_inputs) and all(
                a.shape == b.shape for a, b in zip(micro_batches, g.static_inputs)):
            logs = g.replay(*micro_batches)
        else:
            n = len(micro_batches)
            for x in micro_batches[:-1]:
                self.step_body(x, False, n, None)
            logs = self.step_body(micro_batches[-1], True, n, None)
        self.global_step += len(micro_batches)
        return logs

    def _optim_step(self, opt, red, module):
        if isinstance(opt, FlatAdam):
            opt.step(max_norm=self.max_grad_norm)
            return
        if self.max_grad_norm:
            torch.nn.utils.clip_grad_norm_(module.parameters(), self.max_grad_norm)
        opt.step()
        red.zero_grad()

    def d_phase(self, img, sync=True, accum_steps=1, eta=None, rec=None):
        model, discr = self.model, self.discr
        if rec is None:
            set_requires_grad(model, False)
        set_requires_grad(discr, True)
        self.d_red.begin(sync)
        with self._amp():
            if rec is None:
                rec, _ = model(img)
            d_loss = hinge_d_loss(discr(rec), discr(img)) + self.gradient_penalty(img, rec, eta)
        (d_loss if accum_steps == 1 else d_loss / accum_steps).backward()
        self.d_red.finish()
        if sync:
            self._optim_step(self.d_optim, self.d_red, discr)
        return d_loss.detach()

    def g_phase(self, img, sync=True, accum_steps=1, shared=None):
        model, discr = self.model, self.discr
        set_requires_grad(model, True)
        set_requires_grad(discr, False)
        self.g_red.begin(sync)
        with self._amp():
            rec, codebook_loss = shared if shared is not None else model(img)
            l1 = F.l1_loss(rec, img)
            l2 = F.mse_loss(rec, img)
            g_loss = g_nonsaturating_loss(discr(rec))
            loss = codebook_loss + self.adv_w * g_loss + self.laplace_w * l1 + l2
        (loss if accum_steps == 1 else loss / accum_steps).backward()
        self.g_red.finish()
        if sync:
            self._optim_step(self.g_optim, self.g_red, model)
        return dict(g_loss=g_loss.detach(), l1=l1.detach(), l2=l2.detach(),
                    codebook_loss=codebook_loss.detach(), loss=loss.detach())

    def step_body(self, img, sync=True, accum_steps=1, eta=None):
        shared = None
        if self.share_forward:
            set_requires_grad(self.model, True)
            with self._amp():
                shared = self.model(img)
        d_loss = self.d_phase(img, sync, accum_steps, eta, rec=shared[0].detach() if shared is not None else None)
        logs = self.g_phase(img, sync, accum_steps, shared)
        logs["d_loss"] = d_loss
        return logs

    def save_ckpt(self, path, config=None):
        import torch.distributed as dist

        if dist.is_initialized() and dist.get_rank() != 0:
            return
        ckpt = {"step": self.global_step,
                "state_dict": {k: v.detach().cpu() for k, v in self.model.state_dict().items()},
                "config": config}
        torch.save(ckpt, path)

    def resume_from_checkpoint(self, path):
        import pickle

        try:
            ckpt = torch.load(path, map_location="cpu", weights_only=True)
        except pickle.UnpicklingError as e:
            raise RuntimeError(
                f"{path}: not loadable with weights_only=True ({e}). A reference-written checkpoint must have its "
                "'config' entry converted to a plain dict (or dropped) first; only tensors and plain containers "
                "are loaded here.") from e
        self.global_step = int(ckpt["step"])
        self.model.load_state_dict(ckpt["state_dict"])
        self.g_red.broadcast_parameters()
        if self.fused_optimizer:
            self.g_optim.refresh_shadow()
        return ckpt.get("config")
```

### attention-models_amd/csrc/gemm_x6.hip

```cpp
#include "amk_common.h"

namespace amk_gemm {

typedef __bf16 bf16x8 __attribute__((ext_vector_type(8)));
typedef __bf16 bf16x4 __attribute__((ext_vector_type(4)));

constexpr int BM = 128, BN = 128, BK = 32, NTHR = 512;
constexpr int RS = BK + 8;
constexpr int PLANE = 128 * RS;

__device__ __forceinline__ f32x16 mfmab(bf16x8 a, bf16x8 b, f32x16 c) {
  return __builtin_amdgcn_mfma_f32_32x32x16_bf16(a, b, c, 0, 0, 0);
}

__device__ __forceinline__ void split1(float x, __bf16& h, __bf16& m, __bf16& l) {
  h = (__bf16)x;
  const float r1 = x - (float)h;
  m = (__bf16)r1;
  l = (__bf16)(r1 - (float)m);
}

__device__ __forceinline__ void split4(const float4& x, bf16x4 (&pl)[3]) {
  const float v[4] = {x.x, x.y, x.z, x.w};
#pragma unroll
  for (int j = 0; j < 4; ++j) {
    __bf16 h, m, l;
    split1(v[j], h, m, l);
    pl[0][j] = h; pl[1][j] = m; pl[2][j] = l;
  }
}

__global__ __launch_bounds__(256) void split_planes_kernel(const float* __restrict__ W, int64_t ldw, int R, int K, int Kp,
                                                           __bf16* __restrict__ planes) {
  const int64_t i = (int64_t)blockIdx.x * 256 + threadIdx.x;
  const int kq = Kp / 4;
  if (i >= (int64_t)R * kq) return;
  const int r = (int)(i / kq), k = (int)(i % kq) * 4;
  float4 x = make_float4(0.f, 0.f, 0.f, 0.f);
  if (k < K) x = *reinterpret_cast<const float4*>(W + (int64_t)r * ldw + k);
  bf16x4 pl[3];
  split4(x, pl);
#pragma unroll
  for (int p = 0; p < 3; ++p) *reinterpret_cast<bf16x4*>(planes + ((int64_t)p * R + r) * Kp + k) = pl[p];
}

struct Args {
  const float *A, *bias;
  const __bf16* Bp;
  float* C;
  int M, N, K, Kp;
  int64_t lda, ldc;
};

__global__ __launch_bounds__(NTHR, 4) void gemm_x6_nt_kernel(Args g) {
  __shared__ __attribute__((aligned(16))) __bf16 Ap[3 * PLANE];
  __shared__ __attribute__((aligned(16))) __bf16 Bs[3 * PLANE];
  const int tid = threadIdx.x, lane = tid & 63, wave = __builtin_amdgcn_readfirstlane(tid >> 6);
  const int r = lane & 31, h = lane >> 5;
  const int wm = wave >> 2, wn = wave & 3;
  const int ntn = (g.N + BN - 1) / BN;
  const int wg = xcd_remap(blockIdx.x, gridDim.x);
  const int m0 = (wg / ntn) * BM, n0 = (wg % ntn) * BN;

  const int ar = tid >> 3, ac = (tid & 7) * 4;
  const __amdgpu_buffer_rsrc_t a_rsrc =
      __builtin_amdgcn_make_buffer_rsrc((void*)g.A, 0, (int)(((int64_t)(g.M - 1) * g.lda + g.K) * 4), 0x00020000);
  int aoff[2];
#pragma unroll
  for (int j = 0; j < 2; ++j) {
    const int ra = m0 + ar + 64 * j;
    aoff[j] = ra < g.M ? (int)(((int64_t)ra * g.lda + ac) * 4) : 0x7ffffff0;
  }
  const int br = tid >> 2, bc = (tid & 3) * 8;
  const __amdgpu_buffer_rsrc_t b_rsrc =
      __builtin_amdgcn_make_buffer_rsrc((void*)g.Bp, 0, (int)((int64_t)3 * g.N * g.Kp * 2), 0x00020000);
  int boff[3];
#pragma unroll
  for (int p = 0; p < 3; ++p)
    boff[p] = n0 + br < g.N ? (int)((((int64_t)p * g.N + n0 + br) * g.Kp + bc) * 2) : 0x7ffffff0;

  float4 ast[2];
  uint4 bst[3];
  auto prefetch = [&](int k0) {
    const bool kin = k0 + ac < g.K;
#pragma unroll
    for (int j = 0; j < 2; ++j)
      ast[j] = __builtin_bit_cast(float4, __builtin_amdgcn_raw_buffer_load_b128(a_rsrc, kin ? aoff[j] + k0 * 4 : 0x7ffffff0, 0, 0));
#pragma unroll
    for (int p = 0; p < 3; ++p)
      bst[p] = __builtin_bit_cast(uint4, __builtin_amdgcn_raw_buffer_load_b128(b_rsrc, boff[p] + k0 * 2, 0, 0));
  };
  auto commit = [&]() {
    __builtin_amdgcn_sched_barrier(0);
#pragma unroll
    for (int j = 0; j < 2; ++j) {
      bf16x4 pa[3];
      split4(ast[j], pa);
#pragma unroll
      for (int p = 0; p < 3; ++p) *reinterpret_cast<bf16x4*>(&Ap[p * PLANE + (ar + 64 * j) * RS + ac]) = pa[p];
    }
#pragma unroll
    for (int p = 0; p < 3; ++p) *reinterpret_cast<uint4*>(&Bs[p * PLANE + br * RS + bc]) = bst[p];
  };

  f32x16 acc[2];
#pragma unroll
  for (int i = 0; i < 2; ++i)
#pragma unroll
    for (int t = 0; t < 16; ++t) acc[i][t] = 0.f;

  const int nk = (g.K + BK - 1) / BK;
  prefetch(0);
  for (int kt = 0; kt < nk; ++kt) {
    __syncthreads();
    commit();
    __syncthreads();
    prefetch(min(kt + 1, nk - 1) * BK);
    __builtin_amdgcn_sched_barrier(0);
#pragma unroll
    for (int s = 0; s < 2; ++s) {
      bf16x8 a[2][3], b[3];
#pragma unroll
      for (int p = 0; p < 3; ++p) {
        b[p] = *reinterpret_cast<const bf16x8*>(&Bs[p * PLANE + (32 * wn + r) * RS + 16 * s + 8 * h]);
#pragma unroll
        for (int i = 0; i < 2; ++i)
          a[i][p] = *reinterpret_cast<const bf16x8*>(&Ap[p * PLANE + (64 * wm + 32 * i + r) * RS + 16 * s + 8 * h]);
      }
#pragma unroll
      for (int q = 0; q < 6; ++q) {
        constexpr int PA[6] = {1, 2, 0, 1, 0, 0};
        constexpr int PB[6] = {1, 0, 2, 0, 1, 0};
#pragma unroll
        for (int i = 0; i < 2; ++i) acc[i] = mfmab(a[i][PA[q]], b[PB[q]], acc[i]);
      }
    }
  }
  const int n = n0 + 32 * wn + r;
  if (n < g.N) {
    const float bv = g.bias ? g.bias[n] : 0.f;
#pragma unroll
    for (int i = 0; i < 2; ++i)
#pragma unroll
      for (int t = 0; t < 16; ++t) {
        const int m = m0 + 64 * wm + 32 * i + acc_row(t, h);
        if (m < g.M) g.C[(int64_t)m * g.ldc + n] = acc[i][t] + bv;
      }
  }
}

}

using namespace amk_gemm;

static int padded_k(int K) { return (K + BK - 1) / BK * BK; }

extern "C" int64_t amk_gemm_x6_planes_bytes(int N, int K) {
  if (N <= 0 || K <= 0) return 0;
  return (int64_t)3 * N * padded_k(K) * 2;
}

extern "C" int amk_gemm_x6_split(const float* W, int64_t ldw, int N, int K, void* planes, void* stream) {
  AMK_CHECK_ARG(W && planes, "amk_gemm_x6_split: null pointer");
  AMK_CHECK_ARG(N > 0 && K > 0, "amk_gemm_x6_split: non-positive size");
  AMK_CHECK_SUPPORTED(K % 4 == 0 && ldw % 4 == 0 && ((reinterpret_cast<uintptr_t>(W) | reinterpret_cast<uintptr_t>(planes)) & 15) == 0,
                      "amk_gemm_x6_split: K, ldw multiples of 4 and 16-byte aligned pointers");
  const int Kp = padded_k(K);
  const int64_t n = (int64_t)N * (Kp / 4);
  AMK_CHECK_SUPPORTED((n + 255) / 256 < (1ll << 31), "amk_gemm_x6_split: grid too large");
  hipLaunchKernelGGL(split_planes_kernel, dim3((unsigned)((n + 255) / 256)), dim3(256), 0, static_cast<hipStream_t>(stream),
                     W, ldw, N, K, Kp, static_cast<__bf16*>(planes));
  AMK_CHECK_LAUNCH("amk_gemm_x6_split");
  return AMK_OK;
}

extern "C" int amk_gemm_x6_nt(const float* A, int64_t lda, const void* b_planes, const float* bias,
                              float* C, int64_t ldc, int M, int N, int K, void* stream) {
  AMK_CHECK_ARG(A && b_planes && C, "amk_gemm_x6_nt: null pointer");
  AMK_CHECK_ARG(M > 0 && N > 0 && K > 0, "amk_gemm_x6_nt: non-positive size M=%d N=%d K=%d", M, N, K);
  AMK_CHECK_SUPPORTED(K % 4 == 0 && lda % 4 == 0 &&
                          ((reinterpret_cast<uintptr_t>(A) | reinterpret_cast<uintptr_t>(b_planes)) & 15) == 0,
                      "amk_gemm_x6_nt: K, lda must be multiples of 4 and A, the planes 16-byte aligned");
  AMK_CHECK_SUPPORTED(((int64_t)(M - 1) * lda + K) * 4 < 0x7ffffff0ll && amk_gemm_x6_planes_bytes(N, K) < 0x7ffffff0ll,
                      "amk_gemm_x6_nt: an operand must span < 2 GiB");
  Args g;
  g.A = A; g.Bp = static_cast<const __bf16*>(b_planes); g.bias = bias; g.C = C;
  g.M = M; g.N = N; g.K = K; g.Kp = padded_k(K); g.lda = lda; g.ldc = ldc;
  const int64_t nwg = (int64_t)((M + BM - 1) / BM) * ((N + BN - 1) / BN);
  AMK_CHECK_SUPPORTED(nwg < (1ll << 31), "amk_gemm_x6_nt: grid too large");
  hipLaunchKernelGGL(gemm_x6_nt_kernel, dim3((unsigned)nwg), dim3(NTHR), 0, static_cast<hipStream_t>(stream), g);
  AMK_CHECK_LAUNCH("amk_gemm_x6_nt");
  return AMK_OK;
}
```

### include/amk.h

```cpp
#ifndef AMK_H_
#define AMK_H_

#include <stdint.h>

#ifdef __cplusplus
extern "C" {
#endif

#define AMK_VERSION 140

enum {
  AMK_OK = 0,
  AMK_EINVAL = -1,
  AMK_EUNSUPPORTED = -2,
  AMK_ELAUNCH = -3
};

int amk_version(void);
const char* amk_arch(void);
const char* amk_last_error(void);

int amk_attn_fwd(const float* q, const float* k, const float* v, float* o, float* stats,
                 const uint8_t* key_mask, const uint8_t* causal_mask,
                 int B, int H, int I, int J, int D,
                 int64_t q_sb, int64_t q_st, int64_t q_sh,
                 int64_t k_sb, int64_t k_st, int64_t k_sh,
                 int64_t v_sb, int64_t v_st, int64_t v_sh,
                 int64_t o_sb, int64_t o_st, int64_t o_sh,
                 float scale, void* stream);

int64_t amk_attn_scores_bytes(int B, int H, int I, int J);
int amk_attn_fwd_keep(const float* q, const float* k, const float* v, float* o, float* stats, float* scores,
                      const uint8_t* key_mask, const uint8_t* causal_mask,
                      int B, int H, int I, int J, int D,
                      int64_t q_sb, int64_t q_st, int64_t q_sh,
                      int64_t k_sb, int64_t k_st, int64_t k_sh,
                      int64_t v_sb, int64_t v_st, int64_t v_sh,
                      int64_t o_sb, int64_t o_st, int64_t o_sh,
                      float scale, void* stream);

int64_t amk_attn_fwd_x6_ws_bytes(int B, int H, int J);
int amk_attn_fwd_x6(const float* q, const float* k, const float* v, float* o, float* stats, void* ws,
                    const uint8_t* key_mask, const uint8_t* causal_mask,
                    int B, int H, int I, int J, int D,
                    int64_t q_sb, int64_t q_st, int64_t q_sh,
                    int64_t k_sb, int64_t k_st, int64_t k_sh,
                    int64_t v_sb, int64_t v_st, int64_t v_sh,
                    int64_t o_sb, int64_t o_st, int64_t o_sh,
                    float scale, void* stream);
int amk_attn_fwd_x6_keep(const float* q, const float* k, const float* v, float* o, float* stats, void* ws, float* scores,
                         const uint8_t* key_mask, const uint8_t* causal_mask,
                         int B, int H, int I, int J, int D,
                         int64_t q_sb, int64_t q_st, int64_t q_sh,
                         int64_t k_sb, int64_t k_st, int64_t k_sh,
                         int64_t v_sb, int64_t v_st, int64_t v_sh,
                         int64_t o_sb, int64_t o_st, int64_t o_sh,
                         float scale, void* stream);

int64_t amk_attn_decode_ws_floats(int B, int H, int D, int capacity);
int amk_attn_decode(const float* q, const float* k_new, const float* v_new, float* k_cache, float* v_cache,
                    float* o, float* ws, const int32_t* n_dev, const uint8_t* key_mask,
                    int B, int H, int D, int capacity,
                    int64_t q_sb, int64_t q_sh, int64_t new_sb, int64_t new_sh,
                    int64_t c_sb, int64_t c_st, int64_t c_sh, int64_t o_sb, int64_t o_sh,
                    float scale, void* stream);

int amk_attn_decode_bf16(const void* q, const void* k_new, const void* v_new, void* k_cache, void* v_cache,
                         void* o, float* ws, const int32_t* n_dev, const uint8_t* key_mask,
                         int B, int H, int D, int capacity,
                         int64_t q_sb, int64_t q_sh, int64_t new_sb, int64_t new_sh,
                         int64_t c_sb, int64_t c_st, int64_t c_sh, int64_t o_sb, int64_t o_sh,
                         float scale, void* stream);

int amk_gemm_rows_bf16(const void* x, int64_t ldx, const void* w, int64_t ldw, const float* bias,
                       void* y, int64_t ldy, int M, int N, int K, int out_bf16, void* stream);

#define AMK_ATTN_BWD_DELTA 1
#define AMK_ATTN_BWD_DKDV 2
#define AMK_ATTN_BWD_DQ 4
#define AMK_ATTN_BWD_FUSED 8
#define AMK_ATTN_BWD_ALL 7
#define AMK_ATTN_BWD_FAST 9
#define AMK_ATTN_BWD_KEYS128 16
#define AMK_ATTN_BWD_KEYS256 32
#define AMK_ATTN_BWD_DQ_REPRO 64
#define AMK_ATTN_BWD_FAST_REPRO 73
int64_t amk_attn_bwd_ws_floats(int B, int H, int I, int J, int stages);
int amk_attn_bwd(const float* q, const float* k, const float* v, const float* o,
                 const float* stats, const float* d_o,
                 float* dq, float* dk, float* dv, float* delta_ws,
                 const uint8_t* key_mask, const uint8_t* causal_mask,
                 int B, int H, int I, int J, int D,
                 int64_t q_sb, int64_t q_st, int64_t q_sh,
                 int64_t k_sb, int64_t k_st, int64_t k_sh,
                 int64_t v_sb, int64_t v_st, int64_t v_sh,
                 int64_t o_sb, int64_t o_st, int64_t o_sh,
                 int64_t do_sb, int64_t do_st, int64_t do_sh,
                 int64_t dq_sb, int64_t dq_st, int64_t dq_sh,
                 int64_t dk_sb, int64_t dk_st, int64_t dk_sh,
                 int64_t dv_sb, int64_t dv_st, int64_t dv_sh,
                 float scale, int stages, void* stream);
int amk_attn_bwd_kept(const float* scores, const float* q, const float* k, const float* v, const float* o,
                      const float* stats, const float* d_o,
                      float* dq, float* dk, float* dv, float* delta_ws,
                      const uint8_t* key_mask, const uint8_t* causal_mask,
                      int B, int H, int I, int J, int D,
                      int64_t q_sb, int64_t q_st, int64_t q_sh,
                      int64_t k_sb, int64_t k_st, int64_t k_sh,
                      int64_t v_sb, int64_t v_st, int64_t v_sh,
                      int64_t o_sb, int64_t o_st, int64_t o_sh,
                      int64_t do_sb, int64_t do_st, int64_t do_sh,
                      int64_t dq_sb, int64_t dq_st, int64_t dq_sh,
                      int64_t dk_sb, int64_t dk_st, int64_t dk_sh,
                      int64_t dv_sb, int64_t dv_st, int64_t dv_sh,
                      float scale, int stages, void* stream);

int64_t amk_vq_num_partials(int64_t N);
int amk_vq_padded_codes(int K, int nsplit);
int amk_vq_lookup_fwd(const float* z, const float* codebook, int64_t N, int K, int C, int nsplit,
                      float* en_ws, float* ee_ws, float* pmin_ws, int32_t* pidx_ws,
                      int64_t* idx, float* out, float* zq, float* zn, float* sqerr_partial,
                      void* stream);

int amk_vq_lookup_bwd(const float* z, const float* codebook, const float* zn, const float* zq,
                      const int64_t* idx, const float* g_out, const float* g_loss, float beta,
                      int64_t N, int K, int C, float* dz, float* dcodebook, void* stream);

int amk_vq_lookup_bwd_rows(const float* z, const float* codebook, const float* zn, const float* zq,
                           const int64_t* idx, const float* g_out, const float* g_loss, float beta,
                           int64_t N, int K, int C, float* dz, float* ge_rows, void* stream);

int amk_vq_gather(const int64_t* idx, const float* codebook, int64_t N, int K, int C,
                  float* out, int32_t* bad_count, void* stream);


int64_t amk_moe_route_ws_ints(int64_t U, int E, int k);
int amk_moe_route(const float* logits, int64_t U, int E, int k,
                  int64_t* ids, float* gate, int32_t* counts, int32_t* rank, int32_t* blockhist,
                  int32_t* offsets, int32_t* perm, void* stream);

int amk_grouped_gemm_nt(const float* A, int64_t lda, int a_div, const float* W, const float* bias,
                        const int32_t* offsets, const int32_t* perm, int64_t P, int E, int N, int Kd,
                        float* Y, void* stream);

int amk_grouped_gemm_nn(const float* A, int64_t lda, int a_div, const float* W, const float* scale,
                        const int32_t* offsets, const int32_t* perm, int64_t P, int E, int N, int Kd,
                        float* Y, void* stream);

int amk_grouped_gemm_nt_acc(const float* A, int64_t lda, int a_div, const float* W, const float* bias,
                            const int32_t* offsets, const int32_t* perm, int64_t P, int E, int N, int Kd,
                            float* Y, int y_div, void* stream);
int amk_grouped_gemm_nn_acc(const float* A, int64_t lda, int a_div, const float* W, const float* scale,
                            const int32_t* offsets, const int32_t* perm, int64_t P, int E, int N, int Kd,
                            float* Y, int y_div, void* stream);

int amk_grouped_gemm_wgrad(const float* G, int64_t ldg, int g_div, const float* X, int64_t ldx, int x_div,
                           const float* scale, const int32_t* offsets, const int32_t* perm,
                           int64_t P, int E, int N, int Kd, float* dW, float* dbias, void* stream);

int amk_moe_combine(const float* Y, const int64_t* ids, const float* scale, int64_t G, int outer, int k,
                    int N, float* out, void* stream);

int amk_moe_topk(const float* logits, int64_t U, int E, int k, int64_t* ids, float* gate, void* stream);

int amk_moe_route_distinct(const int64_t* ids, int64_t G, int fan, int E, uint64_t* mask,
                           int32_t* offsets, int32_t* perm, void* stream);

int amk_moe_combine_rows(const float* Y, const int64_t* ids, const float* scale, int64_t G, int outer, int k,
                         int N, int v_div, int E, float* out, void* stream);
int amk_moe_gate_grad_rows(const float* d_out, const float* Y, const int64_t* ids, const float* gate,
                           int64_t P, int k, int E, int N, int g_div, int v_div, float* dlogits, void* stream);

int amk_moe_expert_sums(const float* A, int64_t lda, int a_div, const int64_t* ids, const float* scale,
                        int64_t G, int fan, int E, int d, float* Z, void* stream);

int amk_moe_gate_grad(const float* d_out, const float* Y, const int64_t* ids, const float* gate,
                      int64_t P, int k, int E, int N, int g_div, float* dlogits, void* stream);

int amk_agent_num_chunks(int T);
int64_t amk_agent_ws_floats(int B, int H, int T, int P, int backward);
int amk_agent_num_chunks_dh(int T, int D);
int64_t amk_agent_ws_floats_dh(int B, int H, int T, int P, int D, int backward);

int amk_agent_attn_fwd(const float* q, const float* k, const float* v, const float* conv_w, const float* conv_b,
                       float* o, float* agents, float* vagent, float* stats1, float* ws,
                       int B, int H, int T, int D, int P,
                       int64_t q_sb, int64_t q_st, int64_t q_sh, int64_t k_sb, int64_t k_st, int64_t k_sh,
                       int64_t v_sb, int64_t v_st, int64_t v_sh, int64_t o_sb, int64_t o_st, int64_t o_sh,
                       float scale, void* stream);

int amk_agent_attn_bwd(const float* q, const float* k, const float* v, const float* conv_w, const float* d_o,
                       const float* agents, const float* vagent, const float* stats1,
                       float* dq, float* dk, float* dv, float* ws, float* dconvw_part, float* dconvb_part,
                       int B, int H, int T, int D, int P,
                       int64_t q_sb, int64_t q_st, int64_t q_sh, int64_t k_sb, int64_t k_st, int64_t k_sh,
                       int64_t v_sb, int64_t v_st, int64_t v_sh, int64_t do_sb, int64_t do_st, int64_t do_sh,
                       int64_t dq_sb, int64_t dq_st, int64_t dq_sh, int64_t dk_sb, int64_t dk_st, int64_t dk_sh,
                       int64_t dv_sb, int64_t dv_st, int64_t dv_sh, float scale, void* stream);

int amk_agent_conv_grad_reduce(const float* dconvw_part, const float* dconvb_part, int64_t rows, int D,
                               float* dconvw, float* dconvb, void* stream);

int amk_rowsum_num_partials(int64_t M);
int amk_add_layernorm_fwd(const float* x, const float* res, const float* gamma, const float* beta,
                          int64_t M, int D, float eps, float* h, float* y, float* mean, float* rstd, void* stream);
int amk_add_layernorm_bwd(const float* dy, const float* h, const float* dh_in, const float* gamma,
                          const float* mean, const float* rstd, int64_t M, int D, float* dh, float* dgb_part,
                          void* stream);
int amk_colsum(const float* x, int64_t M, int N, float* part, void* stream);

int amk_swiglu_fwd(const float* ab, int64_t M, int H, float* out, void* stream);
int amk_swiglu_bwd(const float* ab, const float* d_out, int64_t M, int H, float* d_ab, void* stream);

int amk_geglu_fwd(const float* ab, int64_t M, int H, float* out, void* stream);
int amk_geglu_bwd(const float* ab, const float* d_out, int64_t M, int H, float* d_ab, void* stream);

int amk_opt_num_partials(void);
int amk_sumsq_partials(const float* x, int64_t n, float* partials, void* stream);
int amk_adam_flat_step(float* param, float* grad, float* exp_avg, float* exp_avg_sq, int64_t n,
                       const int32_t* seg_param, const float* param_tab,
                       const float* partials, int n_partials,
                       float max_norm, float lr, float beta1, float beta2, float eps, float weight_decay,
                       int decoupled, float* norm_out, void* stream);
int amk_adam_flat_step_shadow(float* param, float* grad, float* exp_avg, float* exp_avg_sq, int64_t n,
                              const int32_t* seg_param, const float* param_tab,
                              const float* partials, int n_partials,
                              float max_norm, float lr, float beta1, float beta2, float eps, float weight_decay,
                              int decoupled, float* norm_out, void* param_bf16, void* stream);

int amk_sample_step(const float* logits, const float* null_logits, float cfg_scale,
                    const float* gumbel, uint64_t seed, uint64_t offset, float tau,
                    int64_t R, int V, int keep, const uint8_t* mask, float unmasked_score,
                    int64_t* ids, float* scores, void* stream);

int64_t amk_gemm_x6_planes_bytes(int N, int K);
int amk_gemm_x6_split(const float* W, int64_t ldw, int N, int K, void* planes, void* stream);
int amk_gemm_x6_nt(const float* A, int64_t lda, const void* w_planes, const float* bias,
                   float* C, int64_t ldc, int M, int N, int K, void* stream);

enum { AMK_GEMM_NT = 0, AMK_GEMM_NN = 1, AMK_GEMM_TN = 2 };
enum { AMK_EPI_BIAS = 0, AMK_EPI_RESID = 1, AMK_EPI_SWIGLU = 2, AMK_EPI_SWIGLU_BWD = 3 };
typedef struct amk_gemm_desc {
  int32_t op, epilogue;
  int64_t m;
  int32_t n, k, split, reserved;
  const float *a, *a2, *w, *w2;
  float *c, *c2;
  int64_t lda, lda2, ldw, ldw2, ldc, ldc2;
  const float *bias, *bias2, *resid;
  int64_t ldr;
  const float *ln_mean, *ln_rstd, *ln_gamma, *ln_beta;
  const float* ab;
  int64_t ldab;
  float* gate;
  int64_t ldg;
  float* dbias;
} amk_gemm_desc;
int64_t amk_gemm_f32_ws_bytes(const amk_gemm_desc* d);
int amk_gemm_f32(const amk_gemm_desc* d, void* workspace, int64_t ws_bytes, void* stream);
int amk_row_stats(const float* x, int64_t M, int D, float eps, float* mean, float* rstd, void* stream);

int amk_attn_bf16_fwd(const void* q, const void* k, const void* v, void* o, float* stats,
                      const uint8_t* key_mask, const uint8_t* causal_mask,
                      int B, int H, int I, int J, int D,
                      int64_t q_sb, int64_t q_st, int64_t q_sh, int64_t k_sb, int64_t k_st, int64_t k_sh,
                      int64_t v_sb, int64_t v_st, int64_t v_sh, int64_t o_sb, int64_t o_st, int64_t o_sh,
                      float scale, void* stream);
int64_t amk_attn_bf16_bwd_ws_floats(int B, int H, int I, int J);
int amk_attn_bf16_bwd(const void* q, const void* k, const void* v, const void* o, const float* stats, const void* d_o,
                      void* dq, void* dk, void* dv, float* ws,
                      const uint8_t* key_mask, const uint8_t* causal_mask,
                      int B, int H, int I, int J, int D,
                      int64_t q_sb, int64_t q_st, int64_t q_sh, int64_t k_sb, int64_t k_st, int64_t k_sh,
                      int64_t v_sb, int64_t v_st, int64_t v_sh, int64_t o_sb, int64_t o_st, int64_t o_sh,
                      int64_t do_sb, int64_t do_st, int64_t do_sh, int64_t dq_sb, int64_t dq_st, int64_t dq_sh,
                      int64_t dk_sb, int64_t dk_st, int64_t dk_sh, int64_t dv_sb, int64_t dv_st, int64_t dv_sh,
                      float scale, void* stream);

int amk_swiglu_bf16_fwd(const void* ab, int64_t M, int H, void* out, void* stream);
int amk_swiglu_bf16_bwd(const void* ab, const void* d_out, int64_t M, int H, void* d_ab, void* stream);
int amk_add_layernorm_mixed_fwd(const void* x, int x_is_bf16, const float* res, const float* gamma, const float* beta,
                                int64_t M, int D, float eps, float* h, void* y_bf16, float* mean, float* rstd, void* stream);
int amk_add_layernorm_mixed_bwd(const void* dy, int dy_is_bf16, const float* h, const float* dh_in, const float* gamma,
                                const float* mean, const float* rstd, int64_t M, int D, float* dh, void* dh_bf16,
                                float* dgb_part, void* stream);

int amk_geglu_ln_bf16_num_partials(int64_t M, int H);
int amk_geglu_ln_bf16_fwd(const void* ab, int64_t ab_stride, int64_t M, int H, const float* gamma, const float* beta,
                          float eps, void* y, float* mean, float* rstd, void* stream);
int amk_geglu_ln_bf16_bwd(const void* ab, int64_t ab_stride, const void* dy, const float* gamma, const float* mean,
                          const float* rstd, int64_t M, int H, void* d_ab, float* dgb_part, void* stream);

int64_t amk_gemm_tn_bf16_ws_bytes(int64_t M, int N, int K);
int amk_gemm_tn_bf16(const void* y, int64_t ldy, const void* x, int64_t ldx, float* c, int64_t ldc, float* dbias,
                     int64_t M, int N, int K, void* workspace, int64_t ws_bytes, void* stream);

int amk_gemm_bf16(int op, int epi, const void* a, int64_t lda, const void* w, int64_t ldw, const float* bias,
                  void* c, int64_t ldc, void* g, int64_t ldg, int64_t M, int N, int K, void* stream);

int amk_gemm_bf16_swiglu_bwd(const void* dy, int64_t lddy, const void* w3, int64_t ldw, const void* ab, int64_t ldab,
                             void* dab, int64_t lddab, int64_t M, int H, int K, void* stream);

int64_t amk_bnact_ws_floats(int N, int C, int64_t HW);
int amk_bnact_fwd(const float* x, const float* gamma, const float* beta, int N, int C, int64_t HW, float eps,
                  float momentum, float slope, float* z, float* mean, float* rstd, float* running_mean,
                  float* running_var, float* ws, void* stream);
int amk_bnact_bwd(const float* gz, const float* x, const float* gamma, const float* beta, const float* mean,
                  const float* rstd, int N, int C, int64_t HW, float slope, float* gx, float* sums, float* dgamma,
                  float* dbeta, float* ws, void* stream);
int amk_bnact_bwd_bwd(const float* ggx, const float* gg_gamma, const float* gg_beta, const float* gz, const float* x,
                      const float* gamma, const float* beta, const float* mean, const float* rstd, const float* sums,
                      int N, int C, int64_t HW, float slope, float* g_gz, float* g_x, float* g_gamma, float* ws,
                      void* stream);

int amk_bnact_bf16_fwd(const void* x, const float* gamma, const float* beta, int N, int C, int64_t HW, float eps,
                       float momentum, float slope, void* z, float* mean, float* rstd, float* running_mean,
                       float* running_var, float* ws, void* stream);
int amk_bnact_bf16_bwd(const void* gz, const void* x, const float* gamma, const float* beta, const float* mean,
                       const float* rstd, int N, int C, int64_t HW, float slope, void* gx, float* sums, float* dgamma,
                       float* dbeta, float* ws, void* stream);
int amk_bnact_bf16_bwd_bwd(const void* ggx, const float* gg_gamma, const float* gg_beta, const void* gz, const void* x,
                           const float* gamma, const float* beta, const float* mean, const float* rstd,
                           const float* sums, int N, int C, int64_t HW, float slope, void* g_gz, void* g_x,
                           float* g_gamma, float* ws, void* stream);

int64_t amk_gnact_ws_floats(int N, int C, int64_t HW, int G);
int amk_gnact_fwd(const float* x, const float* gamma, const float* beta, int N, int C, int64_t HW, int G, float eps,
                  int act, float* z, float* mean, float* rstd, float* ws, void* stream);
int amk_gnact_bwd(const float* gz, const float* x, const float* gamma, const float* beta, const float* mean,
                  const float* rstd, int N, int C, int64_t HW, int G, int act, float* gx, float* dgamma, float* dbeta,
                  float* ws, void* stream);

int64_t amk_gnact_bf16_ws_floats(int N, int C, int64_t HW, int G);
int amk_gnact_bf16_fwd(const void* x, const float* gamma, const float* beta, int N, int C, int64_t HW, int G, float eps,
                       int act, void* z, float* mean, float* rstd, float* ws, void* stream);
int amk_gnact_bf16_bwd(const void* gz, const void* x, const float* gamma, const float* beta, const float* mean,
                       const float* rstd, int N, int C, int64_t HW, int G, int act, void* gx, float* dgamma, float* dbeta,
                       float* ws, void* stream);

int64_t amk_ce_head_fwd_ws_bytes(int64_t M, int V, int K);
int64_t amk_ce_head_bwd_ws_bytes(int64_t M, int V, int K);
int amk_ce_head_fwd(const float* x, int64_t ldx, const float* w, int64_t ldw, const int64_t* target,
                    int64_t ignore_index, int64_t M, int V, int K, float* loss, float* lse, int32_t* rows,
                    int32_t* count, void* ws, int64_t ws_bytes, void* stream);
int amk_ce_head_bwd(const float* x, int64_t ldx, const float* w, int64_t ldw, const int64_t* target,
                    int64_t ignore_index, int64_t M, int V, int K, const float* d_loss, const float* lse,
                    const int32_t* rows, const int32_t* count, float* dx, int64_t lddx, float* dw, int64_t lddw,
                    void* ws, int64_t ws_bytes, void* stream);

int amk_ce_head_bias_fwd(const float* x, int64_t ldx, const float* w, int64_t ldw, const float* bias,
                         const int64_t* target, int64_t ignore_index, int64_t M, int V, int K, float* loss, float* lse,
                         int32_t* rows, int32_t* count, void* ws, int64_t ws_bytes, void* stream);
int amk_ce_head_bias_bwd(const float* x, int64_t ldx, const float* w, int64_t ldw, const float* bias,
                         const int64_t* target, int64_t ignore_index, int64_t M, int V, int K, const float* d_loss,
                         const float* lse, const int32_t* rows, const int32_t* count, float* dx, int64_t lddx, float* dw,
                         int64_t lddw, float* dbias, void* ws, int64_t ws_bytes, void* stream);

int64_t amk_ce_head_bf16_fwd_ws_bytes(int64_t M, int V, int K);
int64_t amk_ce_head_bf16_bwd_ws_bytes(int64_t M, int V, int K);
int amk_ce_head_bf16_fwd(const void* x, int64_t ldx, const void* w, int64_t ldw, const int64_t* target,
                         int64_t ignore_index, int64_t M, int V, int K, float* loss, float* lse, int32_t* rows,
                         int32_t* count, void* ws, int64_t ws_bytes, void* stream);
int amk_ce_head_bf16_bwd(const void* x, int64_t ldx, const void* w, int64_t ldw, const int64_t* target,
                         int64_t ignore_index, int64_t M, int V, int K, const float* d_loss, const float* lse,
                         const int32_t* rows, const int32_t* count, void* dx, int64_t lddx, float* dw, int64_t lddw,
                         void* ws, int64_t ws_bytes, void* stream);

int amk_ce_head_bias_bf16_fwd(const void* x, int64_t ldx, const void* w, int64_t ldw, const float* bias,
                              const int64_t* target, int64_t ignore_index, int64_t M, int V, int K, float* loss, float* lse,
                              int32_t* rows, int32_t* count, void* ws, int64_t ws_bytes, void* stream);
int amk_ce_head_bias_bf16_bwd(const void* x, int64_t ldx, const void* w, int64_t ldw, const float* bias,
                              const int64_t* target, int64_t ignore_index, int64_t M, int V, int K, const float* d_loss,
                              const float* lse, const int32_t* rows, const int32_t* count, void* dx, int64_t lddx, float* dw,
                              int64_t lddw, float* dbias, void* ws, int64_t ws_bytes, void* stream);

int amk_grouped_gemm_nt_bf16(const void* A, int64_t lda, int a_div, const void* W, const float* bias,
                             const int32_t* offsets, const int32_t* perm, int64_t P, int E, int N, int Kd,
                             float* Y, void* stream);
int amk_grouped_gemm_nn_bf16(const void* G, int64_t ldg, int a_div, const void* W, const float* scale,
                             const int32_t* offsets, const int32_t* perm, int64_t P, int E, int N, int Kd,
                             float* Y, void* stream);
int amk_grouped_gemm_wgrad_bf16(const void* G, int64_t ldg, int g_div, const void* X, int64_t ldx, int x_div,
                                const float* scale, const int32_t* offsets, const int32_t* perm,
                                int64_t P, int E, int N, int Kd, float* dW, float* dbias, void* stream);

int amk_grouped_gemm_nt64_bf16(const void* A, int64_t lda, int a_div, const void* W, const float* bias,
                               const int32_t* offsets, const int32_t* perm, int64_t P, int E, int N, int Kd,
                               float* Y, void* stream);
int amk_grouped_gemm_nn64_bf16(const void* G, int64_t ldg, int a_div, const void* W, const float* scale,
                               const int32_t* offsets, const int32_t* perm, int64_t P, int E, int N, int Kd,
                               float* Y, void* stream);
int amk_grouped_gemm_wgrad64_bf16(const void* G, int64_t ldg, int g_div, const void* X, int64_t ldx, int x_div,
                                  const float* scale, const int32_t* offsets, const int32_t* perm,
                                  int64_t P, int E, int N, int Kd, float* dW, void* stream);
int amk_moe_expert_sums_bf16(const void* A, int a_is_bf16, int64_t lda, int a_div, const int64_t* ids, const float* scale,
                             int64_t G, int fan, int E, int d, void* Z, void* stream);

#ifdef __cplusplus
}
#endif
#endif
```

Measured before the change: 313.0 images/s.

## Route generator linears and SwiGLU FFN through bf16x6 split-plane GEMMs by default

Switches the default GEMM mode to auto, so the generator's linear, linear2 and SwiGLU FFN forward GEMMs run on bf16x3-plane (x6) matrix-core kernels. The weight planes are pre-split from the flat parameter buffers right after each Adam step. The kernels gain fused SwiGLU gate and SwiGLU-backward epilogues, a two-segment accumulate form, and an optional transposed plane set for dx. This trades extra plane memory and a per-step split kernel for replacing fp32 FMA GEMMs with bf16 matrix instructions that emulate fp32 accuracy. There is some risk around version-stamp staleness and small numeric differences.

```diff
diff --git a/attention-models_amd/amk/dense.py b/attention-models_amd/amk/dense.py
--- a/attention-models_amd/amk/dense.py
+++ b/attention-models_amd/amk/dense.py
@@ -174,6 +174,83 @@
     return dw, dw2, db
 
 
+class X6Planes:
+    __slots__ = ("w", "wt", "gate", "R", "K")
+
+    def __init__(self, w, wt, gate, R, K):
+        self.w, self.wt, self.gate, self.R, self.K = w, wt, gate, R, K
+
+
+def _pad32(n):
+    return -(-n // 32) * 32
+
+
+def x6_split_plan(entries, transposed=True):
+    rows, spans, blk, off = [], [], 0, 0
+    for src, R, K, gate in entries:
+        if R % 4 or K % 4 or R <= 0 or K <= 0 or (gate and R % 2):
+            raise RuntimeError(f"x6 planes: a weight of shape {(R, K)} cannot be split (multiples of 4 required)")
+        H = R // 2 if gate else 0
+        NR = _lib.load().amk_gemm_x6_gate_rows(H) if gate else R
+        nw, nt = 3 * NR * _pad32(K), (3 * K * _pad32(R) if transposed else 0)
+        dst_w, dst_wt = off, -1
+        off += -(-nw // 128) * 128
+        if transposed:
+            dst_wt = off
+            off += -(-nt // 128) * 128
+        rows.append([src, R, K, H, blk, dst_w, dst_wt, NR])
+        spans.append((dst_w, nw, dst_wt, nt))
+        blk += (_pad32(R) // 32) * (_pad32(K) // 32)
+    return torch.tensor(rows, dtype=torch.int64).view(-1, 8), blk, off, spans
+
+
+def x6_split_table(flat, table_dev, n_blocks, planes):
+    rc = _lib.load().amk_gemm_x6_split_table(_p(flat), flat.numel(), _p(table_dev), table_dev.shape[0], n_blocks,
+                                             _p(planes), planes.numel(), _stream())
+    _lib.check(rc, "amk_gemm_x6_split_table")
+
+
+def gemm_x6_nt(a, planes, N, bias=None, *, a2=None, planes2=None):
+    a, a2 = _mat(a, "a"), _mat(a2, "a2")
+    M, K = a.shape
+    c = torch.empty((M, N), device=a.device, dtype=torch.float32)
+    L = _lib.load()
+    if a2 is not None:
+        if bias is not None or a2.shape[0] != M:
+            raise RuntimeError("gemm_x6_nt: the two-segment form takes no bias and equal row counts")
+        rc = L.amk_gemm_x6_nt2(_p(a), a.stride(0), _p(planes), K, _p(a2), a2.stride(0), _p(planes2), a2.shape[1],
+                               _p(c), N, M, N, _stream())
+        _lib.check(rc, "amk_gemm_x6_nt2")
+        return c
+    rc = L.amk_gemm_x6_nt(_p(a), a.stride(0), _p(planes), _p(_vec(bias, N, "bias")), _p(c), N, M, N, K, _stream())
+    _lib.check(rc, "amk_gemm_x6_nt")
+    return c
+
+
+def gemm_x6_nt_swiglu(a, gate_planes, H, b12=None, *, keep_ab=True):
+    a = _mat(a, "a")
+    M, K = a.shape
+    gate = torch.empty((M, H), device=a.device, dtype=torch.float32)
+    ab = torch.empty((M, 2 * H), device=a.device, dtype=torch.float32) if keep_ab else None
+    rc = _lib.load().amk_gemm_x6_nt_swiglu(_p(a), a.stride(0), _p(gate_planes), _p(_vec(b12, 2 * H, "b12")), _p(gate), H,
+                                           _p(ab), 2 * H, M, H, K, _stream())
+    _lib.check(rc, "amk_gemm_x6_nt_swiglu")
+    return gate, ab
+
+
+def gemm_x6_nt_swiglu_bwd(dy, w3t_planes, ab):
+    dy, ab = _mat(dy, "dy"), _mat(ab, "ab")
+    M, K = dy.shape
+    H = ab.shape[1] // 2
+    if ab.shape != (M, 2 * H):
+        raise RuntimeError(f"gemm_x6_nt_swiglu_bwd: (a | b) {tuple(ab.shape)} against dy {tuple(dy.shape)}")
+    d_ab = torch.empty((M, 2 * H), device=dy.device, dtype=torch.float32)
+    rc = _lib.load().amk_gemm_x6_nt_swiglu_bwd(_p(dy), dy.stride(0), _p(w3t_planes), _p(ab), ab.stride(0), _p(d_ab), 2 * H,
+                                               M, H, K, _stream())
+    _lib.check(rc, "amk_gemm_x6_nt_swiglu_bwd")
+    return d_ab
+
+
 def _mat16(t, what):
     if not t.is_cuda:
         raise RuntimeError("amk ops run only on MI355X (HIP) tensors; got a CPU tensor. There is no CPU fallback.")
diff --git a/attention-models_amd/amk/lib.py b/attention-models_amd/amk/lib.py
--- a/attention-models_amd/amk/lib.py
+++ b/attention-models_amd/amk/lib.py
@@ -74,6 +74,11 @@
     "amk_gemm_x6_planes_bytes": (_L, [_I, _I]),
     "amk_gemm_x6_split": (_I, [_P, _L, _I, _I, _P, _P]),
     "amk_gemm_x6_nt": (_I, [_P, _L, _P, _P, _P, _L, _I, _I, _I, _P]),
+    "amk_gemm_x6_nt2": (_I, [_P, _L, _P, _I, _P, _L, _P, _I, _P, _L, _I, _I, _P]),
+    "amk_gemm_x6_gate_rows": (_I, [_I]),
+    "amk_gemm_x6_nt_swiglu": (_I, [_P, _L, _P, _P, _P, _L, _P, _L, _I, _I, _I, _P]),
+    "amk_gemm_x6_nt_swiglu_bwd": (_I, [_P, _L, _P, _P, _L, _P, _L, _I, _I, _I, _P]),
+    "amk_gemm_x6_split_table": (_I, [_P, _L, _P, _I, _L, _P, _L, _P]),
     "amk_gemm_f32_ws_bytes": (_L, [_c.POINTER(GemmDesc)]),
     "amk_gemm_f32": (_I, [_c.POINTER(GemmDesc), _P, _L, _P]),
     "amk_row_stats": (_I, [_P, _L, _I, _F, _P, _P, _P]),
diff --git a/attention-models_amd/amk/ops.py b/attention-models_amd/amk/ops.py
--- a/attention-models_amd/amk/ops.py
+++ b/attention-models_amd/amk/ops.py
@@ -1511,7 +1511,12 @@
         return dx, dw, db
 
 
-GEMM_MODE = os.environ.get("AMK_GEMM", "f32")
+GEMM_MODE = os.environ.get("AMK_GEMM", "auto")
+if GEMM_MODE not in ("auto", "f32", "bf16x6"):
+    raise RuntimeError(f"AMK_GEMM must be auto, f32 or bf16x6 (got {GEMM_MODE!r})")
+X6_LINEAR = os.environ.get("AMK_X6_LINEAR", "1") != "0"
+X6_AUTO_KINDS = frozenset(k for k in os.environ.get("AMK_X6_KINDS", "linear,linear2,ffn").split(",") if k)
+X6_AUTO_FORMS = frozenset(k for k in os.environ.get("AMK_X6_FORMS", "fwd").split(",") if k)
 
 
 def gemm_x6_nt(a2, b2, bias=None):
@@ -1571,6 +1576,119 @@
         return dx, dw, db
 
 
+def _x6_planes(kind, x, *weights, gate=None):
+    if GEMM_MODE != "auto" or not X6_LINEAR or kind not in X6_AUTO_KINDS or torch.is_autocast_enabled():
+        return None
+    if not x.is_cuda or x.dtype != torch.float32 or x.numel() == 0 or x.shape[-1] % 4:
+        return None
+    if kind == "linear" and min(weights[0].shape) < 128:
+        return None
+    out = []
+    for w in weights:
+        pl = getattr(w, "_amk_x6", None)
+        if pl is None or w._version != w._amk_x6_version or pl.gate != (w is gate) or (pl.R, pl.K) != tuple(w.shape):
+            return None
+        out.append(pl)
+    return tuple(out)
+
+
+class _X6Linear(torch.autograd.Function):
+
+    @staticmethod
+    def forward(ctx, x, weight, bias, pl):
+        from . import dense
+
+        x2 = x.reshape(-1, x.shape[-1])
+        ctx.save_for_backward(x2, weight)
+        ctx.x_shape, ctx.has_bias, ctx.params, ctx.pl = x.shape, bias is not None, (weight, bias), pl
+        return dense.gemm_x6_nt(x2, pl.w, pl.R, bias).view(*x.shape[:-1], pl.R)
+
+    @staticmethod
+    @once_differentiable
+    def backward(ctx, dy):
+        from . import dense
+
+        x2, weight = ctx.saved_tensors
+        dy2 = dy.reshape(-1, dy.shape[-1])
+        dx = dw = db = None
+        if ctx.needs_input_grad[0]:
+            dx = (dense.gemm_x6_nt(dy2, ctx.pl.wt, ctx.pl.K) if ctx.pl.wt is not None else _nn_plain(dy2, weight)).view(ctx.x_shape)
+        if ctx.needs_input_grad[1] or (ctx.has_bias and ctx.needs_input_grad[2]):
+            want_b = ctx.has_bias and ctx.needs_input_grad[2]
+            dw, db = _tn_into(dense.gemm_tn, dy2, x2, ctx.params[0], ctx.params[1] if want_b else None)
+        return dx, dw, db, None
+
+
+class _X6Linear2(torch.autograd.Function):
+
+    @staticmethod
+    def forward(ctx, x, wa, wb, pa, pb):
+        from . import dense
+
+        x2 = x.reshape(-1, x.shape[-1])
+        ctx.save_for_backward(x2, wa, wb)
+        ctx.x_shape, ctx.params, ctx.pl = x.shape, (wa, wb), (pa, pb)
+        a, b = dense.gemm_x6_nt(x2, pa.w, pa.R), dense.gemm_x6_nt(x2, pb.w, pb.R)
+        return a.view(*x.shape[:-1], pa.R), b.view(*x.shape[:-1], pb.R)
+
+    @staticmethod
+    @once_differentiable
+    def backward(ctx, da, db_):
+        from . import dense
+
+        x2, wa, wb = ctx.saved_tensors
+        pa, pb = ctx.pl
+        da2 = da.reshape(-1, da.shape[-1])
+        db2 = db_.reshape(-1, db_.shape[-1])
+        dx = None
+        if ctx.needs_input_grad[0]:
+            dx = (dense.gemm_x6_nt(da2, pa.wt, pa.K, a2=db2, planes2=pb.wt) if pa.wt is not None and pb.wt is not None
+                  else dense.gemm_nn(da2, wa, a2=db2, w2=wb)).view(ctx.x_shape)
+        dwa = dwb = None
+        if ctx.needs_input_grad[1] or ctx.needs_input_grad[2]:
+            (ar, av), (br, bv) = _claim(ctx.params[0]), _claim(ctx.params[1])
+            dwa, dwb, _ = dense.gemm_tn(da2, x2, y2=db2, out=av, out2=bv)
+            if av is not None:
+                ar.wrote(ctx.params[0])
+                dwa = None
+            if bv is not None:
+                br.wrote(ctx.params[1])
+                dwb = None
+        return dx, dwa, dwb, None, None
+
+
+class _X6SwiGLUFFN(torch.autograd.Function):
+
+    @staticmethod
+    def forward(ctx, x, w12, b12, w3, b3, p12, p3):
+        from . import dense
+
+        x2 = x.reshape(-1, x.shape[-1])
+        need = any(ctx.needs_input_grad)
+        gate, ab = dense.gemm_x6_nt_swiglu(x2, p12.w, p12.R // 2, b12, keep_ab=need)
+        out = dense.gemm_x6_nt(gate, p3.w, p3.R, b3)
+        if need:
+            ctx.save_for_backward(x2, w12, w3, ab, gate)
+        ctx.x_shape, ctx.has_bias, ctx.params, ctx.pl = x.shape, (b12 is not None, b3 is not None), (w12, b12, w3, b3), (p12, p3)
+        return out.view(*x.shape[:-1], p3.R)
+
+    @staticmethod
+    @once_differentiable
+    def backward(ctx, dout):
+        from . import dense
+
+        x2, w12, w3, ab, gate = ctx.saved_tensors
+        p12, p3 = ctx.pl
+        d2 = dout.reshape(-1, dout.shape[-1])
+        d_ab = dense.gemm_x6_nt_swiglu_bwd(d2, p3.wt, ab) if p3.wt is not None else dense.gemm_nn(d2, w3, swiglu_ab=ab)
+        dw3, db3 = _tn_into(dense.gemm_tn, d2, gate, ctx.params[2], ctx.params[3] if ctx.has_bias[1] else None)
+        dx = None
+        if ctx.needs_input_grad[0]:
+            dx = (dense.gemm_x6_nt(d_ab, p12.wt, p12.K) if p12.wt is not None else _nn_plain(d_ab, w12)).view(ctx.x_shape)
+        dw12, db12 = _tn_into(dense.gemm_tn, d_ab, x2, ctx.params[0], ctx.params[1] if ctx.has_bias[0] else None)
+        return dx, dw12, db12, dw3, db3, None, None
+
+
 DENSE_MODE = os.environ.get("AMK_DENSE", "auto")
 
 
@@ -1768,6 +1886,9 @@
         return torch.nn.functional.linear(x, weight, bias)
     if GEMM_MODE == "bf16x6" and _x6_ok(x, weight):
         return _LinearX6.apply(x, weight, bias)
+    pl = _x6_planes("linear", x, weight)
+    if pl is not None:
+        return _X6Linear.apply(x, weight, bias, pl[0])
     if _dense_ok(x, weight):
         return _DenseLinear.apply(x, weight, bias)
     if bias is None:
@@ -1776,6 +1897,9 @@
 
 
 def linear2(x, wa, wb):
+    pl = _x6_planes("linear2", x, wa, wb) if wa.shape[0] % 128 == 0 else None
+    if pl is not None:
+        return _X6Linear2.apply(x, wa, wb, *pl)
     if GEMM_MODE != "bf16x6" and _dense_ok(x, wa, wb) and wa.shape[0] % 128 == 0:
         return _DenseLinear2.apply(x, wa, wb)
     return linear(x, wa), linear(x, wb)
@@ -1823,6 +1947,9 @@
 
             g, _ = dense.gemm_nt_swiglu_bf16(x.to(torch.bfloat16).reshape(-1, x.shape[-1]), _w16(w12), b12, keep_ab=False)
             return torch.nn.functional.linear(g, _w16(w3), _w16(b3)).view(*x.shape[:-1], w3.shape[0])
+    pl = _x6_planes("ffn", x, w12, w3, gate=w12) if not torch.is_autocast_enabled() else None
+    if pl is not None:
+        return _X6SwiGLUFFN.apply(x, w12, b12, w3, b3, *pl)
     if GEMM_MODE != "bf16x6" and _dense_ok(x, w12) and w3.shape[1] % 4 == 0 and w3.shape[0] % 4 == 0 and w3.is_contiguous():
         return _SwiGLUFFN.apply(x, w12, b12, w3, b3)
     ab = linear(x, w12, b12)
diff --git a/attention-models_amd/amk/optim.py b/attention-models_amd/amk/optim.py
--- a/attention-models_amd/amk/optim.py
+++ b/attention-models_amd/amk/optim.py
@@ -31,6 +31,7 @@
         skip = {id(p) for p in no_decay}
         self.wd = np.array([0.0 if id(p) in skip else float(weight_decay) for p in self.params], dtype=np.float64)
         self.flat_p, self.m, self.v, self.seg, self.flat_p16 = [], [], [], [], []
+        self.planes = []
         pid = 0
         for b in reducer.buckets:
             fp = torch.zeros_like(b.flat)
@@ -50,6 +51,7 @@
             self.enable_shadow()
         else:
             self.disable_shadow()
+        self.disable_planes()
         self.partials = torch.zeros(len(reducer.buckets) * self.npart, device=dev, dtype=torch.float32)
         self.norm = torch.zeros(1, device=dev, dtype=torch.float32)
         self._tab_host = [torch.zeros(len(self.params), 4).pin_memory() for _ in range(2)]
@@ -79,7 +81,49 @@
             p.__dict__.pop("_amk_bf16_version", None)
         self.flat_p16 = []
 
+    def enable_planes(self, gate=(), transposed=True):
+        from . import dense
+
+        if self.planes and self._planes_t == bool(transposed):
+            return self._split_planes()
+        self.disable_planes()
+        self._planes_t = bool(transposed)
+        gate = {id(p) for p in gate}
+        for b, fp in zip(self.red.buckets, self.flat_p):
+            ent = [(off, p.shape[0], p.shape[1], id(p) in gate, p) for p, off in zip(b.params, b.offsets)
+                   if p.dim() == 2 and p.shape[0] % 4 == 0 and p.shape[1] % 4 == 0]
+            if not ent:
+                self.planes.append(None)
+                continue
+            table, nblk, elems, spans = dense.x6_split_plan([e[:4] for e in ent], transposed=self._planes_t)
+            buf = torch.zeros(elems, device=fp.device, dtype=torch.bfloat16)
+            for (_, R, K, g, p), (dw, nw, dt, nt) in zip(ent, spans):
+                p._amk_x6 = dense.X6Planes(buf[dw:dw + nw], buf[dt:dt + nt] if self._planes_t else None, g, R, K)
+            self.planes.append((buf, table.to(fp.device), nblk, [e[4] for e in ent]))
+        self._split_planes()
+
+    def disable_planes(self):
+        for p in self.params:
+            p.__dict__.pop("_amk_x6", None)
+            p.__dict__.pop("_amk_x6_version", None)
+        self.planes = []
+
+    @property
+    def planes_bytes(self):
+        return sum(pl[0].numel() * 2 for pl in self.planes if pl is not None)
+
+    def _split_planes(self, stamp=True):
+        from . import dense
+
+        for fp, pl in zip(self.flat_p, self.planes):
+            if pl is not None:
+                dense.x6_split_table(fp, pl[1], pl[2], pl[0])
+                if stamp:
+                    for p in pl[3]:
+                        p._amk_x6_version = p._version
+
     def refresh_shadow(self):
+        self._split_planes()
         for fp, f16 in zip(self.flat_p, self.flat_p16):
             f16.copy_(fp)
         if self.flat_p16:
@@ -149,6 +193,7 @@
                 (2 if self.TABLE_WD else 0) | (1 if self.decoupled else 0), _ptr(self.norm) if k == 0 else _ptr(None),
                 _ptr(self.flat_p16[k]) if self.flat_p16 else _ptr(None), stream)
             _lib.check(rc, "amk_adam_flat_step")
+        self._split_planes(stamp=False)
         red.mark_zeroed()
         return self.norm
 
diff --git a/attention-models_amd/amk/train.py b/attention-models_amd/amk/train.py
--- a/attention-models_amd/amk/train.py
+++ b/attention-models_amd/amk/train.py
@@ -266,6 +266,7 @@
             self.g_optim = FlatAdam(self.g_red, lr=lr, betas=betas, weight_decay=weight_decay, capturable=capturable,
                                     bf16_shadow=autocast == torch.bfloat16)
             self.d_optim = FlatAdam(self.d_red, lr=lr, betas=betas, weight_decay=weight_decay, capturable=capturable)
+            self._sync_planes()
         elif capturable:
             dev = next(model.parameters()).device
             okw.update(capturable=True)
@@ -281,6 +282,16 @@
         self.global_step = 0
         self.share_forward = bool(share_forward)
 
+    def _sync_planes(self):
+        from . import ops
+        from .models.vitvqgan import SwiGLU
+
+        if self._autocast is None and ops.GEMM_MODE == "auto" and ops.X6_LINEAR:
+            self.g_optim.enable_planes(gate=[m.w12.weight for m in self.model.modules() if isinstance(m, SwiGLU)],
+                                       transposed="dx" in ops.X6_AUTO_FORMS)
+        else:
+            self.g_optim.disable_planes()
+
     @property
     def autocast(self):
         return self._autocast
@@ -293,6 +304,7 @@
                 self.g_optim.enable_shadow()
             else:
                 self.g_optim.disable_shadow()
+            self._sync_planes()
 
     def _amp(self):
         import contextlib
diff --git a/attention-models_amd/csrc/gemm_x6.hip b/attention-models_amd/csrc/gemm_x6.hip
--- a/attention-models_amd/csrc/gemm_x6.hip
+++ b/attention-models_amd/csrc/gemm_x6.hip
@@ -44,51 +44,79 @@
   for (int p = 0; p < 3; ++p) *reinterpret_cast<bf16x4*>(planes + ((int64_t)p * R + r) * Kp + k) = pl[p];
 }
 
+enum { X6_PLAIN = 0, X6_GATE = 1, X6_GATE_BWD = 2 };
+
 struct Args {
-  const float *A, *bias;
-  const __bf16* Bp;
-  float* C;
-  int M, N, K, Kp;
-  int64_t lda, ldc;
+  const float *A, *A2, *bias, *AB;
+  const __bf16 *Bp, *Bp2;
+  float *C, *G;
+  int M, N, K, Kp, K2, Kp2, NR;
+  int64_t lda, lda2, ldc, ldg, ldab;
 };
 
+__device__ __forceinline__ float sigmoidf_(float x) { return 1.f / (1.f + expf(-x)); }
+
+template <int EPI, bool TWO>
 __global__ __launch_bounds__(NTHR, 4) void gemm_x6_nt_kernel(Args g) {
+  constexpr bool GATE = EPI == X6_GATE;
+  constexpr int TN = GATE ? 64 : BN;
   __shared__ __attribute__((aligned(16))) __bf16 Ap[3 * PLANE];
   __shared__ __attribute__((aligned(16))) __bf16 Bs[3 * PLANE];
   const int tid = threadIdx.x, lane = tid & 63, wave = __builtin_amdgcn_readfirstlane(tid >> 6);
   const int r = lane & 31, h = lane >> 5;
-  const int wm = wave >> 2, wn = wave & 3;
-  const int ntn = (g.N + BN - 1) / BN;
+  const int wm = GATE ? wave >> 1 : wave >> 2, wn = GATE ? wave & 1 : wave & 3;
+  const int ntn = (g.N + TN - 1) / TN;
   const int wg = xcd_remap(blockIdx.x, gridDim.x);
-  const int m0 = (wg / ntn) * BM, n0 = (wg % ntn) * BN;
+  const int m0 = (wg / ntn) * BM, n0 = (wg % ntn) * TN, p0 = (wg % ntn) * BN;
 
   const int ar = tid >> 3, ac = (tid & 7) * 4;
   const __amdgpu_buffer_rsrc_t a_rsrc =
       __builtin_amdgcn_make_buffer_rsrc((void*)g.A, 0, (int)(((int64_t)(g.M - 1) * g.lda + g.K) * 4), 0x00020000);
-  int aoff[2];
+  const __amdgpu_buffer_rsrc_t a2_rsrc = __builtin_amdgcn_make_buffer_rsrc(
+      (void*)(TWO ? g.A2 : g.A), 0, TWO ? (int)(((int64_t)(g.M - 1) * g.lda2 + g.K2) * 4) : 0, 0x00020000);
+  int aoff[2], aoff2[2];
 #pragma unroll
   for (int j = 0; j < 2; ++j) {
     const int ra = m0 + ar + 64 * j;
     aoff[j] = ra < g.M ? (int)(((int64_t)ra * g.lda + ac) * 4) : 0x7ffffff0;
+    aoff2[j] = TWO && ra < g.M ? (int)(((int64_t)ra * g.lda2 + ac) * 4) : 0x7ffffff0;
   }
   const int br = tid >> 2, bc = (tid & 3) * 8;
   const __amdgpu_buffer_rsrc_t b_rsrc =
-      __builtin_amdgcn_make_buffer_rsrc((void*)g.Bp, 0, (int)((int64_t)3 * g.N * g.Kp * 2), 0x00020000);
-  int boff[3];
-#pragma unroll
-  for (int p = 0; p < 3; ++p)
-    boff[p] = n0 + br < g.N ? (int)((((int64_t)p * g.N + n0 + br) * g.Kp + bc) * 2) : 0x7ffffff0;
-
+      __builtin_amdgcn_make_buffer_rsrc((void*)g.Bp, 0, (int)((int64_t)3 * g.NR * g.Kp * 2), 0x00020000);
+  const __amdgpu_buffer_rsrc_t b2_rsrc = __builtin_amdgcn_make_buffer_rsrc(
+      (void*)(TWO ? g.Bp2 : g.Bp), 0, TWO ? (int)((int64_t)3 * g.NR * g.Kp2 * 2) : 0, 0x00020000);
+  int boff[3], boff2[3];
+#pragma unroll
+  for (int p = 0; p < 3; ++p) {
+    boff[p] = p0 + br < g.NR ? (int)((((int64_t)p * g.NR + p0 + br) * g.Kp + bc) * 2) : 0x7ffffff0;
+    boff2[p] = TWO && p0 + br < g.NR ? (int)((((int64_t)p * g.NR + p0 + br) * g.Kp2 + bc) * 2) : 0x7ffffff0;
+  }
+
+  const int nk1 = (g.K + BK - 1) / BK;
+  const int nk = nk1 + (TWO ? (g.K2 + BK - 1) / BK : 0);
   float4 ast[2];
   uint4 bst[3];
-  auto prefetch = [&](int k0) {
-    const bool kin = k0 + ac < g.K;
-#pragma unroll
-    for (int j = 0; j < 2; ++j)
-      ast[j] = __builtin_bit_cast(float4, __builtin_amdgcn_raw_buffer_load_b128(a_rsrc, kin ? aoff[j] + k0 * 4 : 0x7ffffff0, 0, 0));
-#pragma unroll
-    for (int p = 0; p < 3; ++p)
-      bst[p] = __builtin_bit_cast(uint4, __builtin_amdgcn_raw_buffer_load_b128(b_rsrc, boff[p] + k0 * 2, 0, 0));
+  auto prefetch = [&](int kt) {
+    if (TWO && kt >= nk1) {
+      const int k0 = (kt - nk1) * BK;
+      const bool kin = k0 + ac < g.K2;
+#pragma unroll
+      for (int j = 0; j < 2; ++j)
+        ast[j] = __builtin_bit_cast(float4, __builtin_amdgcn_raw_buffer_load_b128(a2_rsrc, kin ? aoff2[j] + k0 * 4 : 0x7ffffff0, 0, 0));
+#pragma unroll
+      for (int p = 0; p < 3; ++p)
+        bst[p] = __builtin_bit_cast(uint4, __builtin_amdgcn_raw_buffer_load_b128(b2_rsrc, boff2[p] + k0 * 2, 0, 0));
+    } else {
+      const int k0 = kt * BK;
+      const bool kin = k0 + ac < g.K;
+#pragma unroll
+      for (int j = 0; j < 2; ++j)
+        ast[j] = __builtin_bit_cast(float4, __builtin_amdgcn_raw_buffer_load_b128(a_rsrc, kin ? aoff[j] + k0 * 4 : 0x7ffffff0, 0, 0));
+#pragma unroll
+      for (int p = 0; p < 3; ++p)
+        bst[p] = __builtin_bit_cast(uint4, __builtin_amdgcn_raw_buffer_load_b128(b_rsrc, boff[p] + k0 * 2, 0, 0));
+    }
   };
   auto commit = [&]() {
     __builtin_amdgcn_sched_barrier(0);
@@ -109,43 +137,126 @@
 #pragma unroll
     for (int t = 0; t < 16; ++t) acc[i][t] = 0.f;
 
-  const int nk = (g.K + BK - 1) / BK;
   prefetch(0);
   for (int kt = 0; kt < nk; ++kt) {
     __syncthreads();
     commit();
     __syncthreads();
-    prefetch(min(kt + 1, nk - 1) * BK);
+    prefetch(min(kt + 1, nk - 1));
     __builtin_amdgcn_sched_barrier(0);
 #pragma unroll
     for (int s = 0; s < 2; ++s) {
-      bf16x8 a[2][3], b[3];
-#pragma unroll
-      for (int p = 0; p < 3; ++p) {
-        b[p] = *reinterpret_cast<const bf16x8*>(&Bs[p * PLANE + (32 * wn + r) * RS + 16 * s + 8 * h]);
-#pragma unroll
-        for (int i = 0; i < 2; ++i)
-          a[i][p] = *reinterpret_cast<const bf16x8*>(&Ap[p * PLANE + (64 * wm + 32 * i + r) * RS + 16 * s + 8 * h]);
+      constexpr int PA[6] = {1, 2, 0, 1, 0, 0};
+      constexpr int PB[6] = {1, 0, 2, 0, 1, 0};
+      if constexpr (GATE) {
+        bf16x8 a[3], b[2][3];
+#pragma unroll
+        for (int p = 0; p < 3; ++p) {
+          a[p] = *reinterpret_cast<const bf16x8*>(&Ap[p * PLANE + (32 * wm + r) * RS + 16 * s + 8 * h]);
+#pragma unroll
+          for (int i = 0; i < 2; ++i)
+            b[i][p] = *reinterpret_cast<const bf16x8*>(&Bs[p * PLANE + (64 * i + 32 * wn + r) * RS + 16 * s + 8 * h]);
+        }
+#pragma unroll
+        for (int q = 0; q < 6; ++q)
+#pragma unroll
+          for (int i = 0; i < 2; ++i) acc[i] = mfmab(a[PA[q]], b[i][PB[q]], acc[i]);
+      } else {
+        bf16x8 a[2][3], b[3];
+#pragma unroll
+        for (int p = 0; p < 3; ++p) {
+          b[p] = *reinterpret_cast<const bf16x8*>(&Bs[p * PLANE + (32 * wn + r) * RS + 16 * s + 8 * h]);
+#pragma unroll
+          for (int i = 0; i < 2; ++i)
+            a[i][p] = *reinterpret_cast<const bf16x8*>(&Ap[p * PLANE + (64 * wm + 32 * i + r) * RS + 16 * s + 8 * h]);
+        }
+#pragma unroll
+        for (int q = 0; q < 6; ++q)
+#pragma unroll
+          for (int i = 0; i < 2; ++i) acc[i] = mfmab(a[i][PA[q]], b[PB[q]], acc[i]);
       }
-#pragma unroll
-      for (int q = 0; q < 6; ++q) {
-        constexpr int PA[6] = {1, 2, 0, 1, 0, 0};
-        constexpr int PB[6] = {1, 0, 2, 0, 1, 0};
-#pragma unroll
-        for (int i = 0; i < 2; ++i) acc[i] = mfmab(a[i][PA[q]], b[PB[q]], acc[i]);
+    }
+  }
+  const int n = n0 + 32 * wn + r;
+  if (n >= g.N) return;
+  if constexpr (GATE) {
+    const float ba = g.bias ? g.bias[n] : 0.f, bb = g.bias ? g.bias[g.N + n] : 0.f;
+#pragma unroll
+    for (int t = 0; t < 16; ++t) {
+      const int m = m0 + 32 * wm + acc_row(t, h);
+      if (m < g.M) {
+        const float av = acc[0][t] + ba, bv = acc[1][t] + bb;
+        g.G[(int64_t)m * g.ldg + n] = av * sigmoidf_(av) * bv;
+        if (g.C) { g.C[(int64_t)m * g.ldc + n] = av; g.C[(int64_t)m * g.ldc + g.N + n] = bv; }
       }
     }
-  }
-  const int n = n0 + 32 * wn + r;
-  if (n < g.N) {
-    const float bv = g.bias ? g.bias[n] : 0.f;
+  } else {
+    const float bv = (EPI == X6_PLAIN && g.bias) ? g.bias[n] : 0.f;
 #pragma unroll
     for (int i = 0; i < 2; ++i)
 #pragma unroll
       for (int t = 0; t < 16; ++t) {
         const int m = m0 + 64 * wm + 32 * i + acc_row(t, h);
-        if (m < g.M) g.C[(int64_t)m * g.ldc + n] = acc[i][t] + bv;
+        if (m < g.M) {
+          if constexpr (EPI == X6_GATE_BWD) {
+            const float dg = acc[i][t], a_ = g.AB[(int64_t)m * g.ldab + n], b_ = g.AB[(int64_t)m * g.ldab + g.N + n];
+            const float sg = sigmoidf_(a_);
+            g.C[(int64_t)m * g.ldc + n] = dg * b_ * (sg * (1.f + a_ * (1.f - sg)));
+            g.C[(int64_t)m * g.ldc + g.N + n] = dg * (a_ * sg);
+          } else {
+            g.C[(int64_t)m * g.ldc + n] = acc[i][t] + bv;
+          }
+        }
       }
+  }
+}
+
+constexpr int SPLIT_ENT = 8;
+
+__global__ __launch_bounds__(256) void split_table_kernel(const float* __restrict__ flat, int64_t flat_elems,
+                                                          const int64_t* __restrict__ table, int n_ent,
+                                                          __bf16* __restrict__ planes, int64_t planes_elems) {
+  __shared__ __bf16 T[3][32][36];
+  const int tid = threadIdx.x;
+  int e = 0;
+  while (e + 1 < n_ent && (int64_t)blockIdx.x >= table[(e + 1) * SPLIT_ENT + 4]) ++e;
+  const int64_t* t = table + e * SPLIT_ENT;
+  const int64_t src = t[0], dst_w = t[5], dst_wt = t[6];
+  const int R = (int)t[1], K = (int)t[2], H = (int)t[3], NR = (int)t[7];
+  const int Kp = (K + 31) / 32 * 32, Rp = (R + 31) / 32 * 32, tk_n = Kp / 32;
+  const int tile = (int)((int64_t)blockIdx.x - t[4]);
+  const int tr = tile / tk_n, tk = tile - tr * tk_n;
+  if (tile < 0 || tr >= Rp / 32 || src < 0 || src + (int64_t)R * K > flat_elems || dst_w < 0 ||
+      dst_w + (int64_t)3 * NR * Kp > planes_elems || (dst_wt >= 0 && dst_wt + (int64_t)3 * K * Rp > planes_elems) ||
+      (H > 0 ? (R != 2 * H || NR < (H + 63) / 64 * 128) : NR < R))
+    return;
+  const int lr = tid >> 3, lc = (tid & 7) * 4;
+  const int rr = 32 * tr + lr, k = 32 * tk + lc;
+  float4 x = make_float4(0.f, 0.f, 0.f, 0.f);
+  if (rr < R && k < K) x = *reinterpret_cast<const float4*>(flat + src + (int64_t)rr * K + k);
+  bf16x4 pl[3];
+  split4(x, pl);
+  if (rr < R) {
+    int pr = rr;
+    if (H > 0) { const int j = rr < H ? rr : rr - H; pr = 128 * (j >> 6) + (j & 63) + (rr < H ? 0 : 64); }
+#pragma unroll
+    for (int p = 0; p < 3; ++p) *reinterpret_cast<bf16x4*>(planes + dst_w + ((int64_t)p * NR + pr) * Kp + k) = pl[p];
+  }
+  if (dst_wt < 0) return;
+#pragma unroll
+  for (int p = 0; p < 3; ++p)
+#pragma unroll
+    for (int j = 0; j < 4; ++j) T[p][lc + j][lr] = pl[p][j];
+  __syncthreads();
+  const int kk = 32 * tk + lr, rc = 32 * tr + lc;
+  if (kk < K) {
+#pragma unroll
+    for (int p = 0; p < 3; ++p) {
+      bf16x4 v;
+#pragma unroll
+      for (int j = 0; j < 4; ++j) v[j] = T[p][lr][lc + j];
+      *reinterpret_cast<bf16x4*>(planes + dst_wt + ((int64_t)p * K + kk) * Rp + rc) = v;
+    }
   }
 }
 
@@ -174,21 +285,76 @@
   return AMK_OK;
 }
 
+static int x6_launch(const char* who, int epi, const float* A, int64_t lda, const void* planes, int K, const float* A2,
+                     int64_t lda2, const void* planes2, int K2, const float* bias, const float* AB, int64_t ldab, float* C,
+                     int64_t ldc, float* G, int64_t ldg, int M, int N, void* stream) {
+  const bool two = A2 != nullptr;
+  AMK_CHECK_ARG(A && planes, "%s: null pointer", who);
+  AMK_CHECK_ARG(M > 0 && N > 0 && K > 0 && (!two || (K2 > 0 && planes2)), "%s: non-positive size M=%d N=%d K=%d", who, M, N, K);
+  AMK_CHECK_SUPPORTED(K % 4 == 0 && lda % 4 == 0 && ((reinterpret_cast<uintptr_t>(A) | reinterpret_cast<uintptr_t>(planes)) & 15) == 0,
+                      "%s: K, lda must be multiples of 4 and A, the planes 16-byte aligned", who);
+  const int NR = epi == X6_GATE ? (N + 63) / 64 * 128 : N;
+  AMK_CHECK_SUPPORTED(((int64_t)(M - 1) * lda + K) * 4 < 0x7ffffff0ll && (int64_t)3 * NR * padded_k(K) * 2 < 0x7ffffff0ll,
+                      "%s: an operand must span < 2 GiB", who);
+  if (two) {
+    AMK_CHECK_SUPPORTED(K2 % 4 == 0 && lda2 % 4 == 0 && ((reinterpret_cast<uintptr_t>(A2) | reinterpret_cast<uintptr_t>(planes2)) & 15) == 0,
+                        "%s: K2, lda2 must be multiples of 4 and A2, its planes 16-byte aligned", who);
+    AMK_CHECK_SUPPORTED(((int64_t)(M - 1) * lda2 + K2) * 4 < 0x7ffffff0ll && (int64_t)3 * NR * padded_k(K2) * 2 < 0x7ffffff0ll,
+                        "%s: an operand must span < 2 GiB", who);
+  }
+  Args g;
+  g.A = A; g.A2 = A2; g.bias = bias; g.AB = AB; g.C = C; g.G = G;
+  g.Bp = static_cast<const __bf16*>(planes); g.Bp2 = static_cast<const __bf16*>(planes2);
+  g.M = M; g.N = N; g.K = K; g.Kp = padded_k(K); g.K2 = two ? K2 : 0; g.Kp2 = two ? padded_k(K2) : 0; g.NR = NR;
+  g.lda = lda; g.lda2 = lda2; g.ldc = ldc; g.ldg = ldg; g.ldab = ldab;
+  const int tn = epi == X6_GATE ? 64 : BN;
+  const int64_t nwg = (int64_t)((M + BM - 1) / BM) * ((N + tn - 1) / tn);
+  AMK_CHECK_SUPPORTED(nwg < (1ll << 31), "%s: grid too large", who);
+  const dim3 grid((unsigned)nwg), blk(NTHR);
+  hipStream_t st = static_cast<hipStream_t>(stream);
+  if (epi == X6_GATE) hipLaunchKernelGGL((gemm_x6_nt_kernel<X6_GATE, false>), grid, blk, 0, st, g);
+  else if (epi == X6_GATE_BWD) hipLaunchKernelGGL((gemm_x6_nt_kernel<X6_GATE_BWD, false>), grid, blk, 0, st, g);
+  else if (two) hipLaunchKernelGGL((gemm_x6_nt_kernel<X6_PLAIN, true>), grid, blk, 0, st, g);
+  else hipLaunchKernelGGL((gemm_x6_nt_kernel<X6_PLAIN, false>), grid, blk, 0, st, g);
+  AMK_CHECK_LAUNCH(who);
+  return AMK_OK;
+}
+
 extern "C" int amk_gemm_x6_nt(const float* A, int64_t lda, const void* b_planes, const float* bias,
                               float* C, int64_t ldc, int M, int N, int K, void* stream) {
-  AMK_CHECK_ARG(A && b_planes && C, "amk_gemm_x6_nt: null pointer");
-  AMK_CHECK_ARG(M > 0 && N > 0 && K > 0, "amk_gemm_x6_nt: non-positive size M=%d N=%d K=%d", M, N, K);
-  AMK_CHECK_SUPPORTED(K % 4 == 0 && lda % 4 == 0 &&
-                          ((reinterpret_cast<uintptr_t>(A) | reinterpret_cast<uintptr_t>(b_planes)) & 15) == 0,
-                      "amk_gemm_x6_nt: K, lda must be multiples of 4 and A, the planes 16-byte aligned");
-  AMK_CHECK_SUPPORTED(((int64_t)(M - 1) * lda + K) * 4 < 0x7ffffff0ll && amk_gemm_x6_planes_bytes(N, K) < 0x7ffffff0ll,
-                      "amk_gemm_x6_nt: an operand must span < 2 GiB");
-  Args g;
-  g.A = A; g.Bp = static_cast<const __bf16*>(b_planes); g.bias = bias; g.C = C;
-  g.M = M; g.N = N; g.K = K; g.Kp = padded_k(K); g.lda = lda; g.ldc = ldc;
-  const int64_t nwg = (int64_t)((M + BM - 1) / BM) * ((N + BN - 1) / BN);
-  AMK_CHECK_SUPPORTED(nwg < (1ll << 31), "amk_gemm_x6_nt: grid too large");
-  hipLaunchKernelGGL(gemm_x6_nt_kernel, dim3((unsigned)nwg), dim3(NTHR), 0, static_cast<hipStream_t>(stream), g);
-  AMK_CHECK_LAUNCH("amk_gemm_x6_nt");
+  AMK_CHECK_ARG(C, "amk_gemm_x6_nt: null pointer");
+  return x6_launch("amk_gemm_x6_nt", X6_PLAIN, A, lda, b_planes, K, nullptr, 0, nullptr, 0, bias, nullptr, 0, C, ldc, nullptr, 0, M, N, stream);
+}
+
+extern "C" int amk_gemm_x6_nt2(const float* A, int64_t lda, const void* planes, int K, const float* A2, int64_t lda2,
+                               const void* planes2, int K2, float* C, int64_t ldc, int M, int N, void* stream) {
+  AMK_CHECK_ARG(C && A2 && planes2, "amk_gemm_x6_nt2: null pointer");
+  return x6_launch("amk_gemm_x6_nt2", X6_PLAIN, A, lda, planes, K, A2, lda2, planes2, K2, nullptr, nullptr, 0, C, ldc, nullptr, 0, M, N, stream);
+}
+
+extern "C" int amk_gemm_x6_gate_rows(int H) { return H > 0 ? (H + 63) / 64 * 128 : 0; }
+
+extern "C" int amk_gemm_x6_nt_swiglu(const float* A, int64_t lda, const void* gate_planes, const float* bias, float* gate,
+                                     int64_t ldg, float* ab, int64_t ldab, int M, int H, int K, void* stream) {
+  AMK_CHECK_ARG(gate, "amk_gemm_x6_nt_swiglu: null pointer");
+  return x6_launch("amk_gemm_x6_nt_swiglu", X6_GATE, A, lda, gate_planes, K, nullptr, 0, nullptr, 0, bias, nullptr, 0, ab, ldab, gate, ldg, M, H, stream);
+}
+
+extern "C" int amk_gemm_x6_nt_swiglu_bwd(const float* dY, int64_t ldy, const void* w3t_planes, const float* ab, int64_t ldab,
+                                         float* d_ab, int64_t ldd, int M, int H, int K, void* stream) {
+  AMK_CHECK_ARG(ab && d_ab, "amk_gemm_x6_nt_swiglu_bwd: null pointer");
+  return x6_launch("amk_gemm_x6_nt_swiglu_bwd", X6_GATE_BWD, dY, ldy, w3t_planes, K, nullptr, 0, nullptr, 0, nullptr, ab, ldab, d_ab, ldd, nullptr, 0, M, H, stream);
+}
+
+extern "C" int amk_gemm_x6_split_table(const float* flat, int64_t flat_elems, const void* table, int n_entries, int64_t n_blocks,
+                                       void* planes, int64_t planes_elems, void* stream) {
+  AMK_CHECK_ARG(flat && table && planes, "amk_gemm_x6_split_table: null pointer");
+  AMK_CHECK_ARG(n_entries > 0 && n_blocks > 0 && flat_elems > 0 && planes_elems > 0, "amk_gemm_x6_split_table: non-positive size");
+  AMK_CHECK_SUPPORTED(((reinterpret_cast<uintptr_t>(flat) | reinterpret_cast<uintptr_t>(planes) | reinterpret_cast<uintptr_t>(table)) & 15) == 0,
+                      "amk_gemm_x6_split_table: 16-byte aligned pointers");
+  AMK_CHECK_SUPPORTED(n_blocks < (1ll << 31), "amk_gemm_x6_split_table: grid too large");
+  hipLaunchKernelGGL(split_table_kernel, dim3((unsigned)n_blocks), dim3(256), 0, static_cast<hipStream_t>(stream), flat, flat_elems,
+                     static_cast<const int64_t*>(table), n_entries, static_cast<__bf16*>(planes), planes_elems);
+  AMK_CHECK_LAUNCH("amk_gemm_x6_split_table");
   return AMK_OK;
 }
diff --git a/include/amk.h b/include/amk.h
--- a/include/amk.h
+++ b/include/amk.h
@@ -237,6 +237,15 @@
 int amk_gemm_x6_split(const float* W, int64_t ldw, int N, int K, void* planes, void* stream);
 int amk_gemm_x6_nt(const float* A, int64_t lda, const void* w_planes, const float* bias,
                    float* C, int64_t ldc, int M, int N, int K, void* stream);
+int amk_gemm_x6_nt2(const float* A, int64_t lda, const void* planes, int K, const float* A2, int64_t lda2,
+                    const void* planes2, int K2, float* C, int64_t ldc, int M, int N, void* stream);
+int amk_gemm_x6_gate_rows(int H);
+int amk_gemm_x6_nt_swiglu(const float* A, int64_t lda, const void* gate_planes, const float* bias, float* gate,
+                          int64_t ldg, float* ab, int64_t ldab, int M, int H, int K, void* stream);
+int amk_gemm_x6_nt_swiglu_bwd(const float* dY, int64_t ldy, const void* w3t_planes, const float* ab, int64_t ldab,
+                              float* d_ab, int64_t ldd, int M, int H, int K, void* stream);
+int amk_gemm_x6_split_table(const float* flat, int64_t flat_elems, const void* table, int n_entries, int64_t n_blocks,
+                            void* planes, int64_t planes_elems, void* stream);
 
 enum { AMK_GEMM_NT = 0, AMK_GEMM_NN = 1, AMK_GEMM_TN = 2 };
 enum { AMK_EPI_BIAS = 0, AMK_EPI_RESID = 1, AMK_EPI_SWIGLU = 2, AMK_EPI_SWIGLU_BWD = 3 };
```

Result: faster. 319.7 images/s (median of 6 runs) (+2.2%).
